# maxwellsh/DIGDriver

Hardware: NVIDIA B200
Metric: genome_bases_scanned_per_s (higher is better)
Workload: dtype u8 bases -> int32 counts; f64 p-values

## Files before the change

digdriver_b200/_lib.py:

```python
import ctypes
import os

_PKG_DIR = os.path.dirname(os.path.abspath(__file__))
LIB_PATH = os.environ.get("DIG_LIB_PATH") or os.path.join(_PKG_DIR, "libdigb200.so")

_c = ctypes
_P = _c.c_void_p
_I64 = _c.c_int64
_I = _c.c_int
_U64 = _c.c_uint64
_D = _c.c_double

SIGNATURES = {
    "dig_version": (_I, []),
    "dig_last_error": (_c.c_char_p, []),
    "dig_device_sm_count": (_I, []),
    "dig_packed_words": (_I64, [_I64]),
    "dig_nmask_words": (_I64, [_I64]),
    "dig_pack_genome": (_I, [_P, _I64, _P, _P, _P, _P]),
    "dig_scan_workspace_bytes": (_I64, [_I64]),
    "dig_count_contexts": (_I, [_P, _P, _I64, _P, _P, _P, _P, _P, _P, _I64, _I, _I, _P, _P, _P, _P]),
    "dig_count_contexts_fused53": (_I, [_P, _P, _I64, _P, _P, _P, _P, _P, _I64, _P, _P, _P, _P, _P, _P]),
    "dig_narrow_counts_u16": (_I, [_P, _I64, _P, _P, _P]),
    "dig_peer_broadcast": (_I, [_P, _I64, _P, _I, _P]),
    "dig_nmask_fill_runs": (_I, [_P, _I64, _P, _I64, _I64, _P]),
    "dig_nmask_summary": (_I, [_P, _I64, _I64, _P, _P]),
    "dig_tabulate_capacity": (_I64, [_I64]),
    "dig_tabulate_elements_workspace_bytes": (_I64, [_I64]),
    "dig_tabulate_genes_workspace_bytes": (_I64, [_I64]),
    "dig_synth_genome": (_I, [_P, _I64, _I64, _U64, _I, _P]),
    "dig_mutation_contexts": (_I, [_P, _P, _I64, _P, _P, _P, _P, _P, _I64, _I, _I, _P, _P]),
    "dig_substitution_counts": (_I, [_P, _P, _I64, _I, _I, _P, _P]),
    "dig_count_hits": (_I, [_P, _P, _P, _P, _I64, _P, _P, _I64, _P, _P]),
    "dig_tabulate_elements": (_I, [_P, _P, _P, _P, _I64, _P, _P, _P, _P, _I64, _P, _P, _P, _I64, _I64, _P,
                                   _I64, _I64, _I64, _P, _P, _I, _P]),
    "dig_site_counts": (_I, [_P, _P, _I64, _I64, _I, _P, _P]),
    "dig_tabulate_genes": (_I, [_P, _P, _P, _I64, _P, _P, _I64, _I64, _I64, _P, _P, _P, _P]),
    "dig_element_transfer": (_I, [_P, _P, _P, _P, _P, _I64, _I64, _I, _P, _P, _P, _P, _P, _P, _P, _I64, _I, _P,
                                  _P, _P, _I, _I, _P, _P, _P, _P, _P, _P, _P, _P, _P, _P]),
    "dig_nb_pvalue_greater_midp": (_I, [_P, _P, _P, _I64, _P, _P]),
    "dig_nb_burden_test": (_I, [_P, _P, _P, _P, _I64, _P, _P, _P]),
    "dig_fisher_combine2": (_I, [_P, _P, _I64, _P, _P]),
    "dig_sequence_freq": (_I, [_P, _P, _I, _P, _P]),
    "dig_size_ratio": (_I, [_P, _P, _I64, _P, _P]),
    "dig_gene_scale_sums": (_I, [_P, _P, _P, _P, _P, _P, _I64, _I64, _P, _P]),
    "dig_gene_burden_test": (_I, [_P, _P, _P, _P, _P, _P, _I64, _P, _D, _D, _P, _P]),
    "dig_gene_dnds_sel": (_I, [_P, _P, _P, _P, _I64, _P, _P]),
    "dig_selection_coefficient": (_I, [_P, _P, _P, _P, _P, _I64, _P, _P, _P]),
    "dig_window_denominators": (_I, [_P, _P, _I64, _P, _P, _P]),
    "dig_site_test": (_I, [_P, _P, _P, _P, _P, _I64, _I64, _I, _P, _P, _P, _P, _P, _P, _P, _D, _P, _P, _P, _P, _P]),
    "dig_region_prob_norm": (_I, [_P, _P, _I64, _I, _P, _P]),
    "dig_position_obs": (_I, [_P, _I64, _P, _P, _P, _P, _P, _I64, _I, _I, _I, _P, _I64, _P, _P]),
    "dig_position_test": (_I, [_P, _P, _I64, _P, _P, _P, _P, _P, _I64, _I, _I, _P, _P, _P, _P, _I, _P, _P, _P, _P,
                               _P, _P, _P]),
    "dig_nb_pvalue_exact": (_I, [_P, _P, _P, _I64, _P, _P]),
    "dig_nb_pvalue_variant": (_I, [_I, _P, _P, _P, _P, _I64, _P, _P]),
    "dig_loglik": (_I, [_I, _P, _P, _P, _I64, _P, _P]),
    "dig_gene_llr_test": (_I, [_I, _P, _P, _P, _P, _P, _P, _I64, _P, _P]),
    "dig_element_region_counts": (_I, [_P, _P, _P, _P, _P, _I64, _I64, _I, _P, _P, _P, _I64, _I, _P, _P, _P, _P]),
    "dig_element_psum": (_I, [_P, _P, _P, _I64, _P, _P, _P]),
    "dig_overlap_count": (_I, [_P, _P, _P, _I64, _P, _P, _I64, _P, _P]),
    "dig_overlap_fill": (_I, [_P, _P, _P, _I64, _P, _P, _I64, _P, _P, _P, _P]),
    "dig_cds_substitution_table": (_I, [_P, _P, _I64, _P, _P, _I, _P, _P, _P, _P, _P, _I64, _P, _I, _P, _I, _P, _P,
                                        _P, _P]),
    "dig_annotate_snvs": (_I, [_P, _P, _I64, _P, _P, _I, _P, _P, _P, _P, _P, _I64, _P, _I, _P, _I, _P, _P, _P, _P,
                               _I64, _P, _P, _P]),
}



class ScanOpts(ctypes.Structure):
    _fields_ = [("workspace_d", _c.c_void_p), ("workspace_bytes", _c.c_int64), ("variant", _c.c_int32),
                ("totals_limit_kb", _c.c_uint32), ("tile_window", _c.c_int64), ("n_peer_counts3", _c.c_int32),
                ("nsum_offset_words", _c.c_int32), ("peer_counts3_d", _c.c_void_p * 8), ("mc_counts3_d", _c.c_void_p)]


SCAN_AUTO, SCAN_PER_BASE, SCAN_HEX_PLAIN, SCAN_HEX = 0, 1, 2, 3

_lib = None

KERNELS_PER_CALL = {
    "dig_pack_genome": 1, "dig_count_contexts": 1, "dig_count_contexts_fused53": 1, "dig_synth_genome": 1, "dig_mutation_contexts": 1,
    "dig_substitution_counts": 1, "dig_count_hits": 1, "dig_tabulate_elements": 3, "dig_tabulate_genes": 2, "dig_site_counts": 1,
    "dig_element_transfer": 1, "dig_nb_pvalue_greater_midp": 1, "dig_nb_burden_test": 1, "dig_fisher_combine2": 1,
    "dig_sequence_freq": 1, "dig_size_ratio": 1, "dig_gene_scale_sums": 1, "dig_gene_burden_test": 2,
    "dig_window_denominators": 1, "dig_site_test": 1, "dig_gene_dnds_sel": 1, "dig_selection_coefficient": 1, "dig_region_prob_norm": 1, "dig_position_obs": 1, "dig_position_test": 1, "dig_nb_pvalue_exact": 1,
    "dig_nb_pvalue_variant": 1, "dig_loglik": 1, "dig_gene_llr_test": 1, "dig_overlap_count": 1, "dig_overlap_fill": 1,
    "dig_element_region_counts": 1, "dig_element_psum": 1, "dig_narrow_counts_u16": 1, "dig_peer_broadcast": 1, "dig_nmask_fill_runs": 1,
    "dig_nmask_summary": 1, "dig_cds_substitution_table": 1, "dig_annotate_snvs": 1,
}
launch_count = 0


class DigError(RuntimeError):
    pass


def load():
    global _lib
    if _lib is not None:
        return _lib
    if not os.path.exists(LIB_PATH):
        raise DigError(
            "libdigb200.so not found at %s: the CUDA extension is required (no CPU fallback). "
            "Build it with `python -m digdriver_b200.build`." % LIB_PATH)
    lib = ctypes.CDLL(LIB_PATH)
    for name, (res, args) in SIGNATURES.items():
        fn = getattr(lib, name)
        fn.restype = res
        fn.argtypes = args
    _lib = lib
    return lib


def check(rc, what=""):
    if rc != 0:
        msg = load().dig_last_error()
        raise DigError("%s failed with code %d: %s" % (what or "libdigb200 call", rc, (msg or b"").decode()))


def call(name, *args):
    global launch_count
    fn = getattr(load(), name)
    check(fn(*args), name)
    launch_count += KERNELS_PER_CALL.get(name, 0)
```

digdriver_b200/csrc/api.cu:

```cuda
#include <stdarg.h>
#include <string.h>

#include "dig_common.cuh"

namespace dig {

static thread_local char g_err[512] = "";

void set_error(const char *fmt, ...)
{
    va_list ap;
    va_start(ap, fmt);
    vsnprintf(g_err, sizeof(g_err), fmt, ap);
    va_end(ap);
}

int sm_count()
{
    static thread_local int cached_dev = -1;
    static thread_local int cached = 0;
    int dev = 0;
    if (cudaGetDevice(&dev) != cudaSuccess) return 148;
    if (dev != cached_dev) {
        int n = 0;
        if (cudaDeviceGetAttribute(&n, cudaDevAttrMultiProcessorCount, dev) != cudaSuccess || n <= 0) n = 148;
        cached = n;
        cached_dev = dev;
    }
    return cached;
}

}

extern "C" {

int dig_version(void) { return 100; }

const char *dig_last_error(void) { return dig::g_err; }

int dig_device_sm_count(void) { return dig::sm_count(); }

}
```

digdriver_b200/csrc/dig_common.cuh:

```cuda
#pragma once
#include <cuda_runtime.h>
#include <stdint.h>
#include <stdio.h>

#include "../../include/dig_b200.h"

namespace dig {

void set_error(const char *fmt, ...);
int sm_count();

#define DIG_CHECK_ARG(cond, msg)                           \
    do {                                                   \
        if (!(cond)) {                                     \
            dig::set_error("%s: %s", __func__, msg);       \
            return DIG_ERR_ARG;                            \
        }                                                  \
    } while (0)

#define DIG_CHECK_LAUNCH()                                                          \
    do {                                                                            \
        cudaError_t e__ = cudaGetLastError();                                       \
        if (e__ != cudaSuccess) {                                                   \
            dig::set_error("%s: CUDA error: %s", __func__, cudaGetErrorString(e__)); \
            return DIG_ERR_CUDA;                                                    \
        }                                                                           \
    } while (0)

#define DIG_CUDA(call)                                                              \
    do {                                                                            \
        cudaError_t e__ = (call);                                                   \
        if (e__ != cudaSuccess) {                                                   \
            dig::set_error("%s: %s failed: %s", __func__, #call, cudaGetErrorString(e__)); \
            return DIG_ERR_CUDA;                                                    \
        }                                                                           \
    } while (0)

__host__ __device__ __forceinline__ uint64_t mix64(uint64_t z)
{
    z += 0x9E3779B97F4A7C15ull;
    z = (z ^ (z >> 30)) * 0xBF58476D1CE4E5B9ull;
    z = (z ^ (z >> 27)) * 0x94D049BB133111EBull;
    return z ^ (z >> 31);
}

}
```

digdriver_b200/csrc/genetest.cu:

```cuda
#include <cooperative_groups.h>

#include "nb_math.cuh"

namespace {

using namespace dig_nb;

constexpr int SUMS_CLUSTER = 8;
__global__ void __cluster_dims__(SUMS_CLUSTER, 1, 1) __launch_bounds__(1024) gene_scale_sums_kernel(
    const double *__restrict__ mu, const double *__restrict__ sigma, const double *__restrict__ P,
    const double *__restrict__ pi_indel, const int64_t *__restrict__ obs, const uint8_t *__restrict__ cgc,
    int64_t tp53, int64_t n, double *__restrict__ sums)
{
    __shared__ double sh[3][1024];
    cooperative_groups::cluster_group cluster = cooperative_groups::this_cluster();
    const unsigned int rank = cluster.block_rank();
    double a0 = 0.0, a1 = 0.0, a2 = 0.0;
#pragma unroll 4
    for (int64_t g = (int64_t)rank * 1024 + threadIdx.x; g < n; g += (int64_t)SUMS_CLUSTER * 1024) {
        const double m = mu[g], s = sigma[g];
        const double t0 = m * P[g * 4 + 0];
        if (g != tp53 && !isnan(t0)) a0 += t0;
        if (cgc == nullptr || !cgc[g]) {
            const double alpha = (m * m) / (s * s);
            const double theta = (s * s) / m;
            const double t1 = pi_indel[g] * alpha * theta;
            if (!isnan(t1)) a1 += t1;
            a2 += (double)obs[g * 5 + 4];
        }
    }
    sh[0][threadIdx.x] = a0;
    sh[1][threadIdx.x] = a1;
    sh[2][threadIdx.x] = a2;
    __syncthreads();
    for (int o = 512; o > 0; o >>= 1) {
        if (threadIdx.x < o) {
            sh[0][threadIdx.x] += sh[0][threadIdx.x + o];
            sh[1][threadIdx.x] += sh[1][threadIdx.x + o];
            sh[2][threadIdx.x] += sh[2][threadIdx.x + o];
        }
        __syncthreads();
    }
    cluster.sync();
    if (rank == 0 && threadIdx.x < 3) {
        double acc = 0.0;
        for (unsigned int r = 0; r < (unsigned int)SUMS_CLUSTER; ++r) acc += *cluster.map_shared_rank(&sh[threadIdx.x][0], r);
        sums[threadIdx.x] = acc;
    }
    cluster.sync();
}

__global__ void __launch_bounds__(128) gene_test_kernel(
    const double *__restrict__ mu, const double *__restrict__ sigma, const double *__restrict__ P,
    const double *__restrict__ pi_indel, const int64_t *__restrict__ obs, const int64_t *__restrict__ nsamp,
    int64_t n, const double *__restrict__ sums, double n_syn,
    double scale_factor, double *__restrict__ out)
{
    const int64_t stride = (int64_t)gridDim.x * blockDim.x;
    const double cj = isnan(scale_factor) ? (isnan(n_syn) ? sums[3] : n_syn) / sums[0] : scale_factor;
    const double t_indel = sums[2] / sums[1];
    for (int64_t i = (int64_t)blockIdx.x * blockDim.x + threadIdx.x; i < n * 13; i += stride) {
        const int t = (int)(i / n);
        const int64_t g = i - (int64_t)t * n;
        const double m = mu[g], s = sigma[g];
        const double alpha = (m * m) / (s * s);
        const double theta0 = (s * s) / m;
        const double p_syn = P[g * 4 + 0], p_mis = P[g * 4 + 1], p_nons = P[g * 4 + 2], p_spl = P[g * 4 + 3];
        const double p_trunc = p_nons + p_spl;
        const double p_nonsyn = p_mis + p_trunc;
        double pi, k, theta;
        if (t == 12) {
            pi = pi_indel[g];
            k = (double)obs[g * 5 + 4];
            theta = theta0 * t_indel;
        } else {
            const int c = t % 6;
            pi = c == 0 ? p_syn : c == 1 ? p_mis : c == 2 ? p_nons : c == 3 ? p_spl : c == 4 ? p_trunc : p_nonsyn;
            theta = theta0 * cj;
            if (t < 6) {
                const double o0 = (double)obs[g * 5 + 0], o1 = (double)obs[g * 5 + 1], o2 = (double)obs[g * 5 + 2],
                             o3 = (double)obs[g * 5 + 3];
                k = c == 0 ? o0 : c == 1 ? o1 : c == 2 ? o2 : c == 3 ? o3 : c == 4 ? o2 + o3 : o1 + (o2 + o3);
            } else {
                k = (double)nsamp[g * 7 + (c < 4 ? c : c)];
            }
        }
        const double expv = __dmul_rn(__dmul_rn(alpha, theta), pi);
        const double p = __ddiv_rn(1.0, __dadd_rn(__dmul_rn(theta, pi), 1.0));
        const double pval = nb_midp(k, alpha, p);
        if (t < 6) {
            out[(int64_t)t * n + g] = expv;
            out[(int64_t)(6 + t) * n + g] = pval;
        } else if (t < 12) {
            out[(int64_t)(6 + t) * n + g] = pval;
        } else {
            out[18 * n + g] = expv;
            out[19 * n + g] = pval;
        }
        if (t == 0) {
            out[21 * n + g] = alpha;
            out[22 * n + g] = theta;
            out[23 * n + g] = theta0 * t_indel;
            out[24 * n + g] = pi_indel[g];
            out[25 * n + g] = p_trunc;
            out[26 * n + g] = p_nonsyn;
        }
    }
}

__global__ void __launch_bounds__(256) gene_fisher_kernel(int64_t n, double *__restrict__ out)
{
    const int64_t stride = (int64_t)gridDim.x * blockDim.x;
    for (int64_t g = (int64_t)blockIdx.x * blockDim.x + threadIdx.x; g < n; g += stride)
        out[20 * n + g] = fisher2(out[(6 + 4) * n + g], out[19 * n + g]);
}

__global__ void __launch_bounds__(256) seq_freq_kernel(const unsigned long long *__restrict__ counts,
                                                       const unsigned long long *__restrict__ totals, int n_sub,
                                                       double *__restrict__ freq)
{
    const int j = blockIdx.x * blockDim.x + threadIdx.x;
    if (j < n_sub) freq[j] = (double)counts[j] / (double)totals[j / 3];
}

__global__ void __launch_bounds__(256) size_ratio_kernel(const int64_t *__restrict__ num, const int64_t *__restrict__ den, int64_t n,
                                                         double *__restrict__ out)
{
    const int64_t i = (int64_t)blockIdx.x * blockDim.x + threadIdx.x;
    if (i < n) out[i] = __ddiv_rn((double)num[i], (double)den[i]);
}

}

extern "C" {

int dig_size_ratio(const int64_t *num_d, const int64_t *den_d, int64_t n, double *out_d, void *stream)
{
    DIG_CHECK_ARG(n >= 0, "negative size");
    if (n == 0) return DIG_OK;
    DIG_CHECK_ARG(num_d && den_d && out_d, "null pointer");
    size_ratio_kernel<<<(unsigned)((n + 255) / 256), 256, 0, (cudaStream_t)stream>>>(num_d, den_d, n, out_d);
    DIG_CHECK_LAUNCH();
    return DIG_OK;
}

int dig_sequence_freq(const unsigned long long *subst_counts_d, const unsigned long long *ctx_totals_d, int n_ctx,
                      double *freq_d, void *stream)
{
    DIG_CHECK_ARG(n_ctx > 0 && subst_counts_d && ctx_totals_d && freq_d, "bad arguments");
    const int n_sub = 3 * n_ctx;
    seq_freq_kernel<<<(n_sub + 255) / 256, 256, 0, (cudaStream_t)stream>>>(subst_counts_d, ctx_totals_d, n_sub, freq_d);
    DIG_CHECK_LAUNCH();
    return DIG_OK;
}

int dig_gene_scale_sums(const double *mu_d, const double *sigma_d, const double *p_d, const double *pi_indel_d,
                        const int64_t *obs_d, const uint8_t *cgc_mask_d, int64_t tp53, int64_t n_gene,
                        double *sums_d, void *stream)
{
    DIG_CHECK_ARG(n_gene >= 0 && sums_d, "bad arguments");
    DIG_CHECK_ARG(n_gene == 0 || (mu_d && sigma_d && p_d && pi_indel_d && obs_d), "null pointer");
    gene_scale_sums_kernel<<<SUMS_CLUSTER, 1024, 0, (cudaStream_t)stream>>>(mu_d, sigma_d, p_d, pi_indel_d, obs_d, cgc_mask_d,
                                                                 tp53, n_gene, sums_d);
    DIG_CHECK_LAUNCH();
    return DIG_OK;
}

int dig_gene_burden_test(const double *mu_d, const double *sigma_d, const double *p_d, const double *pi_indel_d,
                         const int64_t *obs_d, const int64_t *nsamp_d, int64_t n_gene, const double *sums_d,
                         double n_syn, double scale_factor, double *out_d, void *stream)
{
    DIG_CHECK_ARG(n_gene >= 0, "negative size");
    if (n_gene == 0) return DIG_OK;
    DIG_CHECK_ARG(mu_d && sigma_d && p_d && pi_indel_d && obs_d && nsamp_d && sums_d && out_d, "null pointer");
    cudaStream_t st = (cudaStream_t)stream;
    int64_t blocks = (n_gene * 13 + 127) / 128;
    const int64_t cap = (int64_t)dig::sm_count() * 32;
    if (blocks > cap) blocks = cap;
    gene_test_kernel<<<(unsigned)blocks, 128, 0, st>>>(mu_d, sigma_d, p_d, pi_indel_d, obs_d, nsamp_d, n_gene, sums_d,
                                                       n_syn, scale_factor, out_d);
    DIG_CHECK_LAUNCH();
    gene_fisher_kernel<<<(unsigned)((n_gene + 255) / 256), 256, 0, st>>>(n_gene, out_d);
    DIG_CHECK_LAUNCH();
    return DIG_OK;
}

}

namespace {

using namespace dig_nb;

__device__ inline double ll_nb(double k, double alpha, double theta)
{
    const double p = __ddiv_rn(1.0, __dadd_rn(1.0, theta));
    const double q = 1.0 - p;
    if (isnan(p) || isnan(k) || isnan(alpha)) return __longlong_as_double(0x7ff8000000000000LL);
    if (q <= 0.0) return k == 0.0 ? 0.0 : -INFINITY;
    if (p <= 0.0) return -INFINITY;
    return log_nb_density(k, alpha, p, q);
}

__global__ void __launch_bounds__(128) gene_dnds_sel_kernel(const double *__restrict__ alpha,
                                                            const double *__restrict__ theta,
                                                            const double *__restrict__ pi,
                                                            const double *__restrict__ obs,
                                                            int64_t n, double *__restrict__ out)
{
    const int64_t stride = (int64_t)gridDim.x * blockDim.x;
    for (int64_t g = (int64_t)blockIdx.x * blockDim.x + threadIdx.x; g < n; g += stride) {
        const double a = alpha[g], t = theta[g];
        double P[6], O[6], E[6];
#pragma unroll
        for (int j = 0; j < 6; ++j) {
            P[j] = pi[g * 6 + j];
            O[j] = obs[g * 6 + j];
            E[j] = __dmul_rn(__dmul_rn(a, t), P[j]);
            out[(int64_t)j * n + g] = E[j];
        }
        const double th_syn = __dmul_rn(t, P[0]);
        double tml = __ddiv_rn(__dadd_rn(__dadd_rn(O[0], a), -1.0), __dadd_rn(1.0, __ddiv_rn(1.0, th_syn)));
        if (a <= 1.0) {
            const double lo = __dmul_rn(a, th_syn);
            tml = tml > lo ? tml : lo;
        }
        const double ratio = __ddiv_rn(tml, E[0]);
        const double mrf = ratio > 1e-10 ? ratio : 1e-10;
        out[6 * n + g] = tml;
        out[7 * n + g] = mrf;
#pragma unroll
        for (int j = 0; j < 6; ++j) {
            const double eml = __dmul_rn(E[j], mrf);
            out[(int64_t)(8 + j) * n + g] = eml;
            const double p = __ddiv_rn(1.0, __dadd_rn(__ddiv_rn(eml, a), 1.0));
            out[(int64_t)(14 + j) * n + g] = nb_midp(O[j], a, p);
        }
        const int cls[3] = {0, 1, 4};
        double l0[3], l1[3];
#pragma unroll
        for (int c = 0; c < 3; ++c) {
            const int j = cls[c];
            l0[c] = ll_nb(O[j], a, __dmul_rn(__dmul_rn(t, P[j]), mrf));
            l1[c] = ll_nb(O[j], a, __ddiv_rn(O[j], a));
        }
        const double ll0 = __dadd_rn(__dadd_rn(l0[0], l0[1]), l0[2]);
        const double ll_syn = __dadd_rn(__dadd_rn(l1[0], l0[1]), l0[2]);
        const double ll_mis = __dadd_rn(__dadd_rn(l0[0], l1[1]), l0[2]);
        const double ll_tr = __dadd_rn(__dadd_rn(l0[0], l0[1]), l1[2]);
        const double ll_ns = __dadd_rn(__dadd_rn(l0[0], l1[1]), l1[2]);
        out[20 * n + g] = chi2_sf(-2.0 * (ll0 - ll_syn), 1);
        out[21 * n + g] = chi2_sf(-2.0 * (ll0 - ll_mis), 1);
        out[22 * n + g] = chi2_sf(-2.0 * (ll0 - ll_tr), 1);
        out[23 * n + g] = chi2_sf(-2.0 * (ll0 - ll_ns), 2);
    }
}

__global__ void __launch_bounds__(128) selection_coef_kernel(const double *__restrict__ obs, const double *__restrict__ ex,
                                                             const double *__restrict__ alpha,
                                                             const double *__restrict__ theta,
                                                             const double *__restrict__ pi, int64_t n,
                                                             double *__restrict__ sel, double *__restrict__ pval)
{
    const int64_t stride = (int64_t)gridDim.x * blockDim.x;
    for (int64_t g = (int64_t)blockIdx.x * blockDim.x + threadIdx.x; g < n; g += stride) {
        const double s = __ddiv_rn(__dadd_rn(obs[g], 1e-16), __dadd_rn(ex[g], 1e-16));
        sel[g] = s;
        if (pval) {
            const double tp = __dmul_rn(theta[g], pi[g]);
            const double ll0 = ll_nb(obs[g], alpha[g], tp);
            const double ll1 = ll_nb(obs[g], alpha[g], __dmul_rn(tp, s));
            pval[g] = chi2_sf(-2.0 * (ll0 - ll1), 1);
        }
    }
}

}

extern "C" int dig_gene_dnds_sel(const double *alpha_d, const double *theta_d, const double *pi6_d, const double *obs6_d,
                                 int64_t n_gene, double *out_d, void *stream)
{
    DIG_CHECK_ARG(n_gene >= 0, "negative size");
    if (n_gene == 0) return DIG_OK;
    DIG_CHECK_ARG(alpha_d && theta_d && pi6_d && obs6_d && out_d, "null pointer");
    int64_t blocks = (n_gene + 127) / 128;
    gene_dnds_sel_kernel<<<(unsigned)blocks, 128, 0, (cudaStream_t)stream>>>(alpha_d, theta_d, pi6_d, obs6_d, n_gene,
                                                                            out_d);
    DIG_CHECK_LAUNCH();
    return DIG_OK;
}

extern "C" int dig_selection_coefficient(const double *obs_d, const double *exp_d, const double *alpha_d,
                                         const double *theta_d, const double *pi_d, int64_t n, double *sel_d,
                                         double *pval_d, void *stream)
{
    DIG_CHECK_ARG(n >= 0, "negative size");
    if (n == 0) return DIG_OK;
    DIG_CHECK_ARG(obs_d && exp_d && sel_d, "null pointer");
    DIG_CHECK_ARG(pval_d == nullptr || (alpha_d && theta_d && pi_d), "p-values need alpha, theta and pi");
    int64_t blocks = (n + 127) / 128;
    selection_coef_kernel<<<(unsigned)blocks, 128, 0, (cudaStream_t)stream>>>(obs_d, exp_d, alpha_d, theta_d, pi_d, n,
                                                                             sel_d, pval_d);
    DIG_CHECK_LAUNCH();
    return DIG_OK;
}

namespace {

__global__ void __launch_bounds__(128) gene_llr_kernel(int model, const double *__restrict__ alpha,
                                                       const double *__restrict__ theta,
                                                       const double *__restrict__ pi,
                                                       const double *__restrict__ obs,
                                                       const double *__restrict__ mrfold, const double *__restrict__ t_syn,
                                                       int64_t n, double *__restrict__ out)
{
    const int64_t stride = (int64_t)gridDim.x * blockDim.x;
    for (int64_t g = (int64_t)blockIdx.x * blockDim.x + threadIdx.x; g < n; g += stride) {
        double r[4];
        llr_row(model, alpha[g], theta[g], pi + g * 3, obs + g * 3, mrfold[g], t_syn ? t_syn[g] : 0.0, r);
#pragma unroll
        for (int j = 0; j < 4; ++j) out[(int64_t)j * n + g] = r[j];
    }
}

}

extern "C" int dig_gene_llr_test(int model, const double *alpha_d, const double *theta_d, const double *pi3_d,
                                 const double *obs3_d, const double *mrfold_d, const double *t_syn_d, int64_t n,
                                 double *out_d, void *stream)
{
    DIG_CHECK_ARG(n >= 0, "negative size");
    DIG_CHECK_ARG(model == DIG_LLR_NB || model == DIG_LLR_GAMMA_POISSON, "unknown model");
    if (n == 0) return DIG_OK;
    DIG_CHECK_ARG(alpha_d && theta_d && pi3_d && obs3_d && mrfold_d && out_d, "null pointer");
    DIG_CHECK_ARG(model == DIG_LLR_NB || t_syn_d, "the gamma-Poisson model needs T_SYN");
    int64_t blocks = (n + 127) / 128;
    gene_llr_kernel<<<(unsigned)blocks, 128, 0, (cudaStream_t)stream>>>(model, alpha_d, theta_d, pi3_d, obs3_d, mrfold_d,
                                                                       t_syn_d, n, out_d);
    DIG_CHECK_LAUNCH();
    return DIG_OK;
}
```

digdriver_b200/csrc/mutctx.cu:

```cuda
#include "dig_common.cuh"

namespace {

__global__ void __launch_bounds__(256) mutctx_kernel(
    const uint32_t *__restrict__ p2, const uint32_t *__restrict__ nmask, int64_t last_p, int64_t last_m,
    const int64_t *__restrict__ chrom_off, const int64_t *__restrict__ chrom_len,
    const int32_t *__restrict__ mut_chrom, const int64_t *__restrict__ mut_start,
    const uint8_t *__restrict__ mut_ref, int64_t n_mut, int n_up, int n_down, int32_t *__restrict__ ctx_out)
{
    const int klen = n_up + n_down + 1;
    const int64_t stride = (int64_t)gridDim.x * blockDim.x;
    for (int64_t i = (int64_t)blockIdx.x * blockDim.x + threadIdx.x; i < n_mut; i += stride) {
        const int32_t c = mut_chrom[i];
        const int64_t p = mut_start[i];
        const int64_t L = __ldg(chrom_len + c);
        const int64_t off = __ldg(chrom_off + c);
        int32_t ctx = -1;
        if (p - n_up >= 0 && p + n_down < L) {
            const int64_t f = off + p - n_up;
            const int64_t w = f >> 4, m = f >> 5;
            const unsigned long long pk = ((unsigned long long)__ldg(p2 + w) << 32) | __ldg(p2 + (w < last_p ? w + 1 : last_p));
            const unsigned long long mk = ((unsigned long long)__ldg(nmask + m) << 32) | __ldg(nmask + (m < last_m ? m + 1 : last_m));
            const uint32_t key = (uint32_t)(pk >> (64 - 2 * ((int)(f & 15) + klen))) & ((1u << (2 * klen)) - 1u);
            const uint32_t bad = (uint32_t)(mk >> (64 - ((int)(f & 31) + klen))) & ((1u << klen) - 1u);
            const uint32_t base = (key >> (2 * n_down)) & 3u;
            const bool base_n = ((bad >> n_down) & 1u) != 0u;
            auto mismatch = [&](int64_t row) -> bool {
                const uint32_t ref = mut_ref[row];
                return ref > 3u || base_n || base != ref;
            };
            bool dropped = mismatch(i);
            for (int64_t j = i - 1; !dropped && j >= 0 && mut_chrom[j] == c && mut_start[j] == p; --j)
                dropped = mismatch(j);
            if (!dropped && bad == 0u) ctx = (int32_t)key;
        }
        ctx_out[i] = ctx;
    }
}

__global__ void __launch_bounds__(256) subst_hist_kernel(const int32_t *__restrict__ ctx,
                                                         const uint8_t *__restrict__ alt, int64_t n, int n_down,
                                                         int n_bins, unsigned long long *__restrict__ counts)
{
    extern __shared__ unsigned int sh[];
    for (int k = threadIdx.x; k < n_bins; k += blockDim.x) sh[k] = 0u;
    __syncthreads();
    const int64_t stride = (int64_t)gridDim.x * blockDim.x;
    for (int64_t i = (int64_t)blockIdx.x * blockDim.x + threadIdx.x; i < n; i += stride) {
        const int32_t c = ctx[i];
        const uint32_t a = alt[i];
        if (c < 0 || a > 3u) continue;
        const uint32_t ref = ((uint32_t)c >> (2 * n_down)) & 3u;
        if (a == ref) continue;
        atomicAdd(sh + 3 * c + (int)(a > ref ? a - 1u : a), 1u);
    }
    __syncthreads();
    for (int k = threadIdx.x; k < n_bins; k += blockDim.x)
        if (sh[k]) atomicAdd(counts + k, (unsigned long long)sh[k]);
}

}

extern "C" int dig_substitution_counts(const int32_t *ctx_d, const uint8_t *alt_d, int64_t n, int n_up, int n_down,
                                       unsigned long long *counts_d, void *stream)
{
    DIG_CHECK_ARG(n >= 0, "negative size");
    DIG_CHECK_ARG(n_up >= 0 && n_down >= 0 && n_up + n_down <= 5, "unsupported context size");
    DIG_CHECK_ARG(counts_d != nullptr, "null pointer");
    const int n_bins = 3 << (2 * (n_up + n_down + 1));
    cudaStream_t st = (cudaStream_t)stream;
    DIG_CUDA(cudaMemsetAsync(counts_d, 0, (size_t)n_bins * sizeof(unsigned long long), st));
    if (n == 0) return DIG_OK;
    DIG_CHECK_ARG(ctx_d && alt_d, "null pointer");
    int64_t blocks = (n + 255) / 256;
    const int64_t cap = (int64_t)dig::sm_count() * 4;
    if (blocks > cap) blocks = cap;
    subst_hist_kernel<<<(unsigned)blocks, 256, (size_t)n_bins * sizeof(unsigned int), st>>>(ctx_d, alt_d, n, n_down,
                                                                                          n_bins, counts_d);
    DIG_CHECK_LAUNCH();
    return DIG_OK;
}

extern "C" int dig_mutation_contexts(const uint32_t *packed2_d, const uint32_t *nmask_d, int64_t n_bases,
                                     const int64_t *chrom_off_d, const int64_t *chrom_len_d,
                                     const int32_t *mut_chrom_d, const int64_t *mut_start_d,
                                     const uint8_t *mut_ref_d, int64_t n_mut, int n_up, int n_down,
                                     int32_t *ctx_out_d, void *stream)
{
    DIG_CHECK_ARG(n_mut >= 0 && n_bases >= 0, "negative size");
    DIG_CHECK_ARG(n_up >= 0 && n_down >= 0 && n_up + n_down <= 14, "unsupported context size");
    if (n_mut == 0) return DIG_OK;
    DIG_CHECK_ARG(packed2_d && nmask_d && chrom_off_d && chrom_len_d && mut_chrom_d && mut_start_d && mut_ref_d &&
                      ctx_out_d,
                  "null pointer");
    int64_t blocks = (n_mut + 255) / 256;
    const int64_t cap = (int64_t)dig::sm_count() * 32;
    if (blocks > cap) blocks = cap;
    mutctx_kernel<<<(unsigned)blocks, 256, 0, (cudaStream_t)stream>>>(
        packed2_d, nmask_d, (((n_bases + 31) >> 5) << 1) - 1, ((n_bases + 31) >> 5) - 1, chrom_off_d, chrom_len_d,
        mut_chrom_d, mut_start_d, mut_ref_d, n_mut, n_up, n_down, ctx_out_d);
    DIG_CHECK_LAUNCH();
    return DIG_OK;
}
```

digdriver_b200/csrc/obs.cu:

```cuda
#include "dig_common.cuh"

namespace {

__device__ __forceinline__ int64_t upper_bound_ge(const int64_t *__restrict__ a, int64_t n, int64_t v)
{
    int64_t lo = 0, hi = n;
    while (lo < hi) {
        const int64_t mid = (lo + hi) >> 1;
        if (__ldg(a + mid) < v) lo = mid + 1;
        else hi = mid;
    }
    return lo;
}

template <typename F>
__device__ __forceinline__ void for_each_hit(const int64_t *__restrict__ bks, const int64_t *__restrict__ bke,
                                             const int64_t *__restrict__ pmax, const int32_t *__restrict__ belt,
                                             int64_t n_blk, int64_t ks, int64_t ke, F f)
{
    if (ke <= ks) return;
    const int64_t hi = upper_bound_ge(bks, n_blk, ke);
    for (int64_t idx = hi - 1; idx >= 0; --idx) {
        if (__ldg(pmax + idx) <= ks) break;
        if (__ldg(bke + idx) <= ks) continue;
        const int32_t e = __ldg(belt + idx);
        bool dup = false;
        for (int64_t j = hi - 1; j > idx && !dup; --j) dup = (__ldg(belt + j) == e) && (__ldg(bke + j) > ks);
        if (!dup) f(e);
    }
}

__global__ void __launch_bounds__(256) count_hits_kernel(
    const int64_t *__restrict__ bks, const int64_t *__restrict__ bke, const int64_t *__restrict__ pmax,
    const int32_t *__restrict__ belt, int64_t n_blk, const int64_t *__restrict__ mks,
    const int64_t *__restrict__ mke, int64_t n_mut, unsigned long long *n_hits)
{
    const int64_t stride = (int64_t)gridDim.x * blockDim.x;
    unsigned long long local = 0;
    for (int64_t i = (int64_t)blockIdx.x * blockDim.x + threadIdx.x; i < n_mut; i += stride)
        for_each_hit(bks, bke, pmax, belt, n_blk, mks[i], mke[i], [&](int32_t) { ++local; });
#pragma unroll
    for (int o = 16; o > 0; o >>= 1) local += __shfl_xor_sync(0xffffffffu, local, o);
    if ((threadIdx.x & 31) == 0 && local) atomicAdd(n_hits, local);
}

__device__ __forceinline__ int64_t table_slot(unsigned long long *keys, int64_t capacity, unsigned long long key)
{
    const int64_t mask = capacity - 1;
    int64_t slot = (int64_t)(dig::mix64(key) & (unsigned long long)mask);
    for (int64_t probes = 0; probes < capacity; ++probes) {
        const unsigned long long prev = atomicCAS(keys + slot, 0ull, key);
        if (prev == 0ull || prev == key) return slot;
        slot = (slot + 1) & mask;
    }
    return -1;
}

__global__ void __launch_bounds__(256) elt_insert_kernel(
    const int64_t *__restrict__ bks, const int64_t *__restrict__ bke, const int64_t *__restrict__ pmax,
    const int32_t *__restrict__ belt, int64_t n_blk, const int64_t *__restrict__ mks,
    const int64_t *__restrict__ mke, const int32_t *__restrict__ msample, const uint8_t *__restrict__ mindel,
    int64_t n_mut, unsigned long long *keys, uint32_t *snv, uint32_t *indel, int64_t capacity, int32_t *status)
{
    const int64_t stride = (int64_t)gridDim.x * blockDim.x;
    for (int64_t i = (int64_t)blockIdx.x * blockDim.x + threadIdx.x; i < n_mut; i += stride) {
        const unsigned long long sample = (unsigned long long)(uint32_t)msample[i];
        const bool is_indel = mindel[i] != 0;
        for_each_hit(bks, bke, pmax, belt, n_blk, mks[i], mke[i], [&](int32_t e) {
            const unsigned long long key = (((unsigned long long)(uint32_t)e << 32) | sample) + 1ull;
            const int64_t slot = table_slot(keys, capacity, key);
            if (slot < 0) {
                *status = 1;
                return;
            }
            atomicAdd((is_indel ? indel : snv) + slot, 1u);
        });
    }
}

__global__ void __launch_bounds__(256) elt_sample_totals_kernel(const unsigned long long *__restrict__ keys,
                                                                const uint32_t *__restrict__ snv,
                                                                const uint32_t *__restrict__ indel, int64_t capacity,
                                                                int rows_mode, unsigned long long *sample_tot)
{
    const int64_t stride = (int64_t)gridDim.x * blockDim.x;
    for (int64_t s = (int64_t)blockIdx.x * blockDim.x + threadIdx.x; s < capacity; s += stride) {
        const unsigned long long key = keys[s];
        if (key == 0ull) continue;
        const uint32_t sample = (uint32_t)((key - 1ull) & 0xFFFFFFFFull);
        atomicAdd(sample_tot + sample, rows_mode ? 1ull : (unsigned long long)snv[s] + (unsigned long long)indel[s]);
    }
}

__global__ void __launch_bounds__(256) elt_finalize_kernel(const unsigned long long *__restrict__ keys,
                                                           const uint32_t *__restrict__ snv,
                                                           const uint32_t *__restrict__ indel, int64_t capacity,
                                                           const unsigned long long *__restrict__ sample_tot,
                                                           int64_t max_per_sample, int64_t max_per_elt_sample,
                                                           int64_t n_elt, int64_t *obs)
{
    const int64_t stride = (int64_t)gridDim.x * blockDim.x;
    for (int64_t s = (int64_t)blockIdx.x * blockDim.x + threadIdx.x; s < capacity; s += stride) {
        const unsigned long long key = keys[s];
        if (key == 0ull) continue;
        const uint32_t sample = (uint32_t)((key - 1ull) & 0xFFFFFFFFull);
        const int64_t e = (int64_t)((key - 1ull) >> 32);
        if (e >= n_elt) continue;
        if ((int64_t)sample_tot[sample] > max_per_sample) continue;
        int64_t a = snv[s], b = indel[s];
        if (a > max_per_elt_sample) a = max_per_elt_sample;
        if (b > max_per_elt_sample) b = max_per_elt_sample;
        atomicAdd(reinterpret_cast<unsigned long long *>(obs + 3 * e + 0), 1ull);
        if (a) atomicAdd(reinterpret_cast<unsigned long long *>(obs + 3 * e + 1), (unsigned long long)a);
        if (b) atomicAdd(reinterpret_cast<unsigned long long *>(obs + 3 * e + 2), (unsigned long long)b);
    }
}

__global__ void __launch_bounds__(256) gene_insert_kernel(const int32_t *__restrict__ mgene,
                                                          const int32_t *__restrict__ msample,
                                                          const uint8_t *__restrict__ mclass, int64_t n_mut,
                                                          unsigned long long *keys, uint32_t *cnt, int64_t capacity,
                                                          int32_t *status)
{
    const int64_t stride = (int64_t)gridDim.x * blockDim.x;
    for (int64_t i = (int64_t)blockIdx.x * blockDim.x + threadIdx.x; i < n_mut; i += stride) {
        const uint32_t cls = mclass[i];
        const int32_t g = mgene[i];
        if (cls > 4u || g < 0) continue;
        const unsigned long long key =
            (((unsigned long long)(uint32_t)g << 32) | (unsigned long long)(uint32_t)msample[i]) + 1ull;
        const int64_t slot = table_slot(keys, capacity, key);
        if (slot < 0) {
            *status = 1;
            continue;
        }
        atomicAdd(cnt + slot * 5 + cls, 1u);
    }
}

__global__ void __launch_bounds__(256) gene_finalize_kernel(const unsigned long long *__restrict__ keys,
                                                            const uint32_t *__restrict__ cnt, int64_t capacity,
                                                            int64_t cap_per, int64_t n_gene, int64_t *obs,
                                                            int64_t *nsamp)
{
    const int64_t stride = (int64_t)gridDim.x * blockDim.x;
    for (int64_t s = (int64_t)blockIdx.x * blockDim.x + threadIdx.x; s < capacity; s += stride) {
        const unsigned long long key = keys[s];
        if (key == 0ull) continue;
        const int64_t g = (int64_t)((key - 1ull) >> 32);
        if (g >= n_gene) continue;
        int64_t c[5];
#pragma unroll
        for (int j = 0; j < 5; ++j) c[j] = cnt[s * 5 + j];
#pragma unroll
        for (int j = 0; j < 5; ++j) {
            const int64_t v = c[j] > cap_per ? cap_per : c[j];
            if (v) atomicAdd(reinterpret_cast<unsigned long long *>(obs + 5 * g + j), (unsigned long long)v);
        }
        const bool flags[7] = {c[0] > 0, c[1] > 0, c[2] > 0, c[3] > 0, (c[2] + c[3]) > 0, (c[1] + c[2] + c[3]) > 0,
                               c[4] > 0};
#pragma unroll
        for (int j = 0; j < 7; ++j)
            if (flags[j]) atomicAdd(reinterpret_cast<unsigned long long *>(nsamp + 7 * g + j), 1ull);
    }
}

__global__ void __launch_bounds__(256) site_counts_kernel(const int32_t *__restrict__ elt, const int32_t *__restrict__ sub,
                                                          int64_t n, int64_t n_elt, int n_sub,
                                                          unsigned long long *__restrict__ L)
{
    const int64_t stride = (int64_t)gridDim.x * blockDim.x;
    for (int64_t i = (int64_t)blockIdx.x * blockDim.x + threadIdx.x; i < n; i += stride) {
        const int32_t e = elt[i], j = sub[i];
        if (e >= 0 && e < n_elt && j >= 0 && j < n_sub) atomicAdd(L + (int64_t)e * n_sub + j, 1ull);
    }
}

inline unsigned grid_for(int64_t n)
{
    int64_t blocks = (n + 255) / 256;
    const int64_t cap = (int64_t)dig::sm_count() * 16;
    if (blocks > cap) blocks = cap;
    return (unsigned)(blocks < 1 ? 1 : blocks);
}

__global__ void __launch_bounds__(256) overlap_count_kernel(
    const int64_t *__restrict__ bks, const int64_t *__restrict__ bke, const int64_t *__restrict__ pmax, int64_t n_blk,
    const int64_t *__restrict__ mks, const int64_t *__restrict__ mke, int64_t n_mut, int64_t *__restrict__ n_pairs)
{
    const int64_t stride = (int64_t)gridDim.x * blockDim.x;
    for (int64_t i = (int64_t)blockIdx.x * blockDim.x + threadIdx.x; i < n_mut; i += stride) {
        const int64_t ks = mks[i], ke = mke[i];
        int64_t c = 0;
        if (ke > ks) {
            const int64_t hi = upper_bound_ge(bks, n_blk, ke);
            for (int64_t idx = hi - 1; idx >= 0; --idx) {
                if (__ldg(pmax + idx) <= ks) break;
                c += __ldg(bke + idx) > ks;
            }
        }
        n_pairs[i] = c;
    }
}

__global__ void __launch_bounds__(256) overlap_fill_kernel(
    const int64_t *__restrict__ bks, const int64_t *__restrict__ bke, const int64_t *__restrict__ pmax, int64_t n_blk,
    const int64_t *__restrict__ mks, const int64_t *__restrict__ mke, int64_t n_mut,
    const int64_t *__restrict__ pair_off, int64_t *__restrict__ pair_mut, int64_t *__restrict__ pair_blk)
{
    const int64_t stride = (int64_t)gridDim.x * blockDim.x;
    for (int64_t i = (int64_t)blockIdx.x * blockDim.x + threadIdx.x; i < n_mut; i += stride) {
        const int64_t ks = mks[i], ke = mke[i];
        if (ke <= ks) continue;
        int64_t w = pair_off[i + 1];
        const int64_t hi = upper_bound_ge(bks, n_blk, ke);
        for (int64_t idx = hi - 1; idx >= 0; --idx) {
            if (__ldg(pmax + idx) <= ks) break;
            if (__ldg(bke + idx) <= ks) continue;
            --w;
            pair_mut[w] = i;
            pair_blk[w] = idx;
        }
    }
}

inline bool is_pow2(int64_t v) { return v > 0 && (v & (v - 1)) == 0; }

}

extern "C" {

int64_t dig_tabulate_capacity(int64_t n_pairs)
{
    if (n_pairs < 0) n_pairs = 0;
    int64_t cap = 1024;
    while (cap < 2 * n_pairs + 16) cap <<= 1;
    return cap;
}
int64_t dig_tabulate_elements_workspace_bytes(int64_t n_pairs) { return dig_tabulate_capacity(n_pairs) * 16; }
int64_t dig_tabulate_genes_workspace_bytes(int64_t n_mut) { return dig_tabulate_capacity(n_mut) * 28; }

int dig_count_hits(const int64_t *blk_kstart_d, const int64_t *blk_kend_d, const int64_t *blk_pmax_d,
                   const int32_t *blk_elt_d, int64_t n_blk, const int64_t *mut_kstart_d,
                   const int64_t *mut_kend_d, int64_t n_mut, unsigned long long *n_hits_d, void *stream)
{
    DIG_CHECK_ARG(n_blk >= 0 && n_mut >= 0, "negative size");
    DIG_CHECK_ARG(n_hits_d != nullptr, "null pointer");
    if (n_blk == 0 || n_mut == 0) return DIG_OK;
    DIG_CHECK_ARG(blk_kstart_d && blk_kend_d && blk_pmax_d && blk_elt_d && mut_kstart_d && mut_kend_d, "null pointer");
    count_hits_kernel<<<grid_for(n_mut), 256, 0, (cudaStream_t)stream>>>(blk_kstart_d, blk_kend_d, blk_pmax_d,
                                                                         blk_elt_d, n_blk, mut_kstart_d, mut_kend_d,
                                                                         n_mut, n_hits_d);
    DIG_CHECK_LAUNCH();
    return DIG_OK;
}

int dig_tabulate_elements(const int64_t *blk_kstart_d, const int64_t *blk_kend_d, const int64_t *blk_pmax_d,
                          const int32_t *blk_elt_d, int64_t n_blk, const int64_t *mut_kstart_d,
                          const int64_t *mut_kend_d, const int32_t *mut_sample_d, const uint8_t *mut_isindel_d,
                          int64_t n_mut, unsigned long long *tab_key_d, uint32_t *tab_snv_d, uint32_t *tab_indel_d,
                          int64_t capacity, int64_t n_sample, unsigned long long *sample_tot_d,
                          int64_t max_muts_per_sample, int64_t max_per_elt_per_sample, int64_t n_elt,
                          int64_t *obs_d, int32_t *status_d, int sample_rows_mode, void *stream)
{
    DIG_CHECK_ARG(n_blk >= 0 && n_mut >= 0 && n_elt >= 0 && n_sample >= 0, "negative size");
    DIG_CHECK_ARG(is_pow2(capacity), "capacity must be a power of two");
    DIG_CHECK_ARG(tab_key_d && tab_snv_d && tab_indel_d && status_d, "null pointer");
    DIG_CHECK_ARG((n_elt == 0 || obs_d) && (n_sample == 0 || sample_tot_d), "null pointer");
    cudaStream_t st = (cudaStream_t)stream;
    DIG_CUDA(cudaMemsetAsync(tab_key_d, 0, (size_t)capacity * sizeof(unsigned long long), st));
    DIG_CUDA(cudaMemsetAsync(tab_snv_d, 0, (size_t)capacity * sizeof(uint32_t), st));
    DIG_CUDA(cudaMemsetAsync(tab_indel_d, 0, (size_t)capacity * sizeof(uint32_t), st));
    DIG_CUDA(cudaMemsetAsync(status_d, 0, sizeof(int32_t), st));
    if (n_sample) DIG_CUDA(cudaMemsetAsync(sample_tot_d, 0, (size_t)n_sample * sizeof(unsigned long long), st));
    if (n_elt) DIG_CUDA(cudaMemsetAsync(obs_d, 0, (size_t)n_elt * 3 * sizeof(int64_t), st));
    if (n_blk == 0 || n_mut == 0) return DIG_OK;
    DIG_CHECK_ARG(blk_kstart_d && blk_kend_d && blk_pmax_d && blk_elt_d && mut_kstart_d && mut_kend_d &&
                      mut_sample_d && mut_isindel_d,
                  "null pointer");
    elt_insert_kernel<<<grid_for(n_mut), 256, 0, st>>>(blk_kstart_d, blk_kend_d, blk_pmax_d, blk_elt_d, n_blk,
                                                       mut_kstart_d, mut_kend_d, mut_sample_d, mut_isindel_d, n_mut,
                                                       tab_key_d, tab_snv_d, tab_indel_d, capacity, status_d);
    DIG_CHECK_LAUNCH();
    elt_sample_totals_kernel<<<grid_for(capacity), 256, 0, st>>>(tab_key_d, tab_snv_d, tab_indel_d, capacity,
                                                                 sample_rows_mode, sample_tot_d);
    DIG_CHECK_LAUNCH();
    elt_finalize_kernel<<<grid_for(capacity), 256, 0, st>>>(tab_key_d, tab_snv_d, tab_indel_d, capacity, sample_tot_d,
                                                            max_muts_per_sample, max_per_elt_per_sample, n_elt, obs_d);
    DIG_CHECK_LAUNCH();
    return DIG_OK;
}

int dig_tabulate_genes(const int32_t *mut_gene_d, const int32_t *mut_sample_d, const uint8_t *mut_class_d,
                       int64_t n_mut, unsigned long long *tab_key_d, uint32_t *tab_cnt_d, int64_t capacity,
                       int64_t max_per_gene_per_sample, int64_t n_gene, int64_t *obs_d, int64_t *nsamp_d,
                       int32_t *status_d, void *stream)
{
    DIG_CHECK_ARG(n_mut >= 0 && n_gene >= 0, "negative size");
    DIG_CHECK_ARG(is_pow2(capacity), "capacity must be a power of two");
    DIG_CHECK_ARG(tab_key_d && tab_cnt_d && status_d && (n_gene == 0 || (obs_d && nsamp_d)), "null pointer");
    cudaStream_t st = (cudaStream_t)stream;
    DIG_CUDA(cudaMemsetAsync(tab_key_d, 0, (size_t)capacity * sizeof(unsigned long long), st));
    DIG_CUDA(cudaMemsetAsync(tab_cnt_d, 0, (size_t)capacity * 5 * sizeof(uint32_t), st));
    DIG_CUDA(cudaMemsetAsync(status_d, 0, sizeof(int32_t), st));
    if (n_gene) {
        DIG_CUDA(cudaMemsetAsync(obs_d, 0, (size_t)n_gene * 5 * sizeof(int64_t), st));
        DIG_CUDA(cudaMemsetAsync(nsamp_d, 0, (size_t)n_gene * 7 * sizeof(int64_t), st));
    }
    if (n_mut == 0) return DIG_OK;
    DIG_CHECK_ARG(mut_gene_d && mut_sample_d && mut_class_d, "null pointer");
    gene_insert_kernel<<<grid_for(n_mut), 256, 0, st>>>(mut_gene_d, mut_sample_d, mut_class_d, n_mut, tab_key_d,
                                                        tab_cnt_d, capacity, status_d);
    DIG_CHECK_LAUNCH();
    gene_finalize_kernel<<<grid_for(capacity), 256, 0, st>>>(tab_key_d, tab_cnt_d, capacity,
                                                             max_per_gene_per_sample, n_gene, obs_d, nsamp_d);
    DIG_CHECK_LAUNCH();
    return DIG_OK;
}

int dig_site_counts(const int32_t *site_elt_d, const int32_t *site_sub_d, int64_t n_site, int64_t n_elt, int n_sub,
                    unsigned long long *L_d, void *stream)
{
    DIG_CHECK_ARG(n_site >= 0 && n_elt >= 0 && n_sub > 0, "bad sizes");
    DIG_CHECK_ARG(n_elt == 0 || L_d, "null pointer");
    cudaStream_t st = (cudaStream_t)stream;
    if (n_elt) DIG_CUDA(cudaMemsetAsync(L_d, 0, (size_t)n_elt * n_sub * sizeof(unsigned long long), st));
    if (n_site == 0 || n_elt == 0) return DIG_OK;
    DIG_CHECK_ARG(site_elt_d && site_sub_d, "null pointer");
    site_counts_kernel<<<grid_for(n_site), 256, 0, st>>>(site_elt_d, site_sub_d, n_site, n_elt, n_sub, L_d);
    DIG_CHECK_LAUNCH();
    return DIG_OK;
}

int dig_overlap_count(const int64_t *blk_kstart_d, const int64_t *blk_kend_d, const int64_t *blk_pmax_d, int64_t n_blk,
                      const int64_t *mut_kstart_d, const int64_t *mut_kend_d, int64_t n_mut, int64_t *n_pairs_d,
                      void *stream)
{
    DIG_CHECK_ARG(n_blk >= 0 && n_mut >= 0, "negative size");
    if (n_mut == 0) return DIG_OK;
    DIG_CHECK_ARG(mut_kstart_d && mut_kend_d && n_pairs_d, "null pointer");
    DIG_CHECK_ARG(n_blk == 0 || (blk_kstart_d && blk_kend_d && blk_pmax_d), "null pointer");
    overlap_count_kernel<<<grid_for(n_mut), 256, 0, (cudaStream_t)stream>>>(blk_kstart_d, blk_kend_d, blk_pmax_d, n_blk,
                                                                            mut_kstart_d, mut_kend_d, n_mut, n_pairs_d);
    DIG_CHECK_LAUNCH();
    return DIG_OK;
}

int dig_overlap_fill(const int64_t *blk_kstart_d, const int64_t *blk_kend_d, const int64_t *blk_pmax_d, int64_t n_blk,
                     const int64_t *mut_kstart_d, const int64_t *mut_kend_d, int64_t n_mut, const int64_t *pair_off_d,
                     int64_t *pair_mut_d, int64_t *pair_blk_d, void *stream)
{
    DIG_CHECK_ARG(n_blk >= 0 && n_mut >= 0, "negative size");
    if (n_mut == 0 || n_blk == 0) return DIG_OK;
    DIG_CHECK_ARG(blk_kstart_d && blk_kend_d && blk_pmax_d && mut_kstart_d && mut_kend_d && pair_off_d, "null pointer");
    DIG_CHECK_ARG(pair_mut_d && pair_blk_d, "null pointer");
    overlap_fill_kernel<<<grid_for(n_mut), 256, 0, (cudaStream_t)stream>>>(blk_kstart_d, blk_kend_d, blk_pmax_d, n_blk,
                                                                           mut_kstart_d, mut_kend_d, n_mut, pair_off_d,
                                                                           pair_mut_d, pair_blk_d);
    DIG_CHECK_LAUNCH();
    return DIG_OK;
}

}
```

digdriver_b200/csrc/transfer.cu:

```cuda
#include "dig_common.cuh"

namespace {

constexpr int TW = 4;
constexpr int MAX_COHORT_PER_LANE = 2;

__device__ __forceinline__ double warp_sum(double v)
{
#pragma unroll
    for (int o = 16; o > 0; o >>= 1) v += __shfl_xor_sync(0xffffffffu, v, o);
    return v;
}

__device__ __forceinline__ int revcomp3(int c)
{
    const int b0 = (c >> 4) & 3, b1 = (c >> 2) & 3, b2 = c & 3;
    return ((3 - b2) << 4) | ((3 - b1) << 2) | (3 - b0);
}

__device__ __forceinline__ int64_t floor_div(int64_t a, int64_t b) { return a >= 0 ? a / b : -((-a + b - 1) / b); }
__device__ __forceinline__ int64_t ceil_div(int64_t a, int64_t b) { return a >= 0 ? (a + b - 1) / b : -((-a) / b); }

template <bool RC>
__global__ void __launch_bounds__(TW * 32, 8) transfer_kernel(
    const int32_t *__restrict__ elt_chrom, const int8_t *__restrict__ elt_strand,
    const int64_t *__restrict__ blk_ptr, const int64_t *__restrict__ blk_start,
    const int64_t *__restrict__ blk_end, int64_t n_elt, int64_t window, int n_chrom,
    const int64_t *__restrict__ win_map_off, const int32_t *__restrict__ win_map, const int32_t *__restrict__ win_counts,
    const double *__restrict__ y_pred, const double *__restrict__ stdv, const double *__restrict__ y_true,
    const uint8_t *__restrict__ flag, int64_t n_win, int n_cohort, const double *__restrict__ d_pr,
    const int32_t *__restrict__ blk_counts, const double *__restrict__ L_elt, int n_col, int span_words,
    double *__restrict__ mu_out, double *__restrict__ sigma_out, double *__restrict__ robs_out,
    uint8_t *__restrict__ flag_out, int64_t *__restrict__ r_size, int64_t *__restrict__ elt_size,
    double *__restrict__ p_out, int32_t *__restrict__ n_win_out, int32_t *__restrict__ status,
    int64_t *__restrict__ region_counts_out)
{
    extern __shared__ __align__(16) unsigned char smem_raw[];
    const int lane = threadIdx.x & 31;
    const int warp = threadIdx.x >> 5;
    const size_t per_warp = 128 * sizeof(double) + (size_t)span_words * sizeof(uint32_t);
    double *r64 = reinterpret_cast<double *>(smem_raw + warp * per_warp);
    double *l64 = r64 + 64;
    uint32_t *bitmap = reinterpret_cast<uint32_t *>(l64 + 64);

    const bool l4_aligned = (reinterpret_cast<uintptr_t>(L_elt) & 15u) == 0;
    const int64_t gwarp = (int64_t)blockIdx.x * TW + warp;
    const int64_t nwarps = (int64_t)gridDim.x * TW;

    for (int64_t e = gwarp; e < n_elt; e += nwarps) {
        const int64_t b0 = blk_ptr[e], b1 = blk_ptr[e + 1];
        const int32_t c = elt_chrom[e];
        const bool minus = elt_strand[e] < 0;
        int64_t wmin = INT64_MAX, wmax = INT64_MIN;
        for (int64_t b = b0 + lane; b < b1; b += 32) {
            const int64_t lo = floor_div(blk_start[b], window);
            const int64_t hi = ceil_div(blk_end[b], window);
            if (hi > lo) {
                wmin = lo < wmin ? lo : wmin;
                wmax = hi > wmax ? hi : wmax;
            }
        }
#pragma unroll
        for (int o = 16; o > 0; o >>= 1) {
            const int64_t a = __shfl_xor_sync(0xffffffffu, wmin, o);
            const int64_t b = __shfl_xor_sync(0xffffffffu, wmax, o);
            wmin = a < wmin ? a : wmin;
            wmax = b > wmax ? b : wmax;
        }
        const int64_t span = wmax > wmin ? wmax - wmin : 0;
        const int words = (int)((span + 31) >> 5);
        bool ok = true;
        if (words > span_words) {
            if (lane == 0) atomicMax(status, 3);
            ok = false;
        }
        if (ok) {
            for (int w = lane; w < words; w += 32) bitmap[w] = 0u;
            __syncwarp();
            for (int64_t b = b0 + lane; b < b1; b += 32) {
                const int64_t lo = floor_div(blk_start[b], window) - wmin;
                const int64_t hi = ceil_div(blk_end[b], window) - wmin;
                for (int64_t w = lo; w < hi;) {
                    const int word = (int)(w >> 5);
                    const int bit = (int)(w & 31);
                    const int64_t upto = ((int64_t)(word + 1) << 5) < hi ? ((int64_t)(word + 1) << 5) : hi;
                    const int nbits = (int)(upto - w);
                    const uint32_t m = (nbits >= 32 ? 0xFFFFFFFFu : ((1u << nbits) - 1u)) << bit;
                    atomicOr(bitmap + word, m);
                    w = upto;
                }
            }
            __syncwarp();
        }
        double r_lo = 0.0, r_hi = 0.0;
        double mu[MAX_COHORT_PER_LANE], var[MAX_COHORT_PER_LANE], ro[MAX_COHORT_PER_LANE];
        int fl[MAX_COHORT_PER_LANE];
#pragma unroll
        for (int q = 0; q < MAX_COHORT_PER_LANE; ++q) mu[q] = var[q] = ro[q] = 0.0, fl[q] = 0;
        int nw = 0;
        const bool chrom_ok = c >= 0 && c < n_chrom;
        const int64_t map0 = chrom_ok ? win_map_off[c] : 0;
        const int64_t map_n = chrom_ok ? win_map_off[c + 1] - map0 : 0;
        for (int w = 0; ok && w < words; ++w) {
            const uint32_t bits = bitmap[w];
            const int cnt = __popc(bits);
            if (cnt == 0) continue;
            int32_t my_row = -1;
            if (lane < cnt) {
                const int64_t wi = wmin + ((int64_t)w << 5) + (int64_t)__fns(bits, 0, lane + 1);
                my_row = (wi >= 0 && wi < map_n) ? __ldg(win_map + map0 + wi) : -1;
            }
            if (__any_sync(0xffffffffu, lane < cnt && my_row < 0) && lane == 0) atomicMax(status, 2);
            for (int k0 = 0; k0 < cnt; k0 += 4) {
                int32_t row[4], clo[4], chi[4];
#pragma unroll
                for (int u = 0; u < 4; ++u) {
                    row[u] = k0 + u < cnt ? __shfl_sync(0xffffffffu, my_row, (k0 + u) & 31) : -1;
                    clo[u] = chi[u] = 0;
                    if (row[u] >= 0) {
                        const int32_t *wc = win_counts + (int64_t)row[u] * 64;
                        clo[u] = __ldg(wc + lane);
                        chi[u] = __ldg(wc + lane + 32);
                    }
                }
#pragma unroll
                for (int u = 0; u < 4; ++u) {
                    if (row[u] < 0) continue;
                    ++nw;
                    r_lo += (double)clo[u];
                    r_hi += (double)chi[u];
                }
            }
            if (n_cohort == 1) {
                double yp = 0.0, sd = 0.0, yt = 0.0;
                int fg = 0;
                if (lane < cnt && my_row >= 0) {
                    yp = __ldg(y_pred + my_row);
                    sd = __ldg(stdv + my_row);
                    yt = __ldg(y_true + my_row);
                    fg = __ldg(flag + my_row) != 0;
                }
                for (int k = 0; k < cnt; ++k) {
                    const double a = __shfl_sync(0xffffffffu, yp, k), b = __shfl_sync(0xffffffffu, sd, k);
                    const double t = __shfl_sync(0xffffffffu, yt, k);
                    const int f = __shfl_sync(0xffffffffu, fg, k);
                    if (__shfl_sync(0xffffffffu, my_row, k) < 0) continue;
                    mu[0] += a;
                    var[0] = __dadd_rn(var[0], __dmul_rn(b, b));
                    ro[0] += t;
                    fl[0] |= f;
                }
            } else {
                for (int k = 0; k < cnt; ++k) {
                    const int32_t row = __shfl_sync(0xffffffffu, my_row, k);
                    if (row < 0) continue;
#pragma unroll
                    for (int q = 0; q < MAX_COHORT_PER_LANE; ++q) {
                        const int ci = lane + 32 * q;
                        if (ci < n_cohort) {
                            const int64_t o = (int64_t)ci * n_win + row;
                            const double s = __ldg(stdv + o);
                            mu[q] += __ldg(y_pred + o);
                            var[q] = __dadd_rn(var[q], __dmul_rn(s, s));
                            ro[q] += __ldg(y_true + o);
                            fl[q] |= __ldg(flag + o) != 0;
                        }
                    }
                }
            }
        }
        __syncwarp();
        if (!minus) {
            r64[lane] = r_lo;
            r64[lane + 32] = r_hi;
        } else {
            r64[revcomp3(lane)] = r_lo;
            r64[revcomp3(lane + 32)] = r_hi;
        }
        double l_lo = 0.0, l_hi = 0.0;
        int64_t gene_len = 0;
        if (blk_counts != nullptr) {
            for (int64_t b = b0; b < b1; ++b) {
                l_lo += (double)__ldg(blk_counts + b * 64 + lane);
                l_hi += (double)__ldg(blk_counts + b * 64 + lane + 32);
            }
            l64[lane] = l_lo;
            l64[lane + 32] = l_hi;
        } else {
            for (int64_t b = b0 + lane; b < b1; b += 32) gene_len += blk_end[b] - blk_start[b] + 1;
#pragma unroll
            for (int o = 16; o > 0; o >>= 1) gene_len += __shfl_xor_sync(0xffffffffu, gene_len, o);
        }
        __syncwarp();
        if (RC) {
            region_counts_out[e * 64 + lane] = (int64_t)r64[lane];
            region_counts_out[e * 64 + lane + 32] = (int64_t)r64[lane + 32];
        }
        const double rsum = warp_sum(r_lo + r_hi);
        const double lsum = warp_sum(l_lo + l_hi);

        for (int ci = 0; ci < n_cohort; ++ci) {
            const double *dp = d_pr + (int64_t)ci * 192;
            double part = 0.0;
#pragma unroll
            for (int t = 0; t < 6; ++t) {
                const int j = lane + 32 * t;
                part += __ldg(dp + j) * r64[j / 3];
            }
            const double denom = warp_sum(part);
            double wgt[6];
#pragma unroll
            for (int t = 0; t < 6; ++t) wgt[t] = __ldg(dp + lane + 32 * t) / denom;
            if (blk_counts == nullptr && n_col == 4 && l4_aligned) {
                const double2 *L2 = reinterpret_cast<const double2 *>(L_elt + (int64_t)e * 192 * 4);
                double2 la[6], lb[6];
#pragma unroll
                for (int t = 0; t < 6; ++t) {
                    la[t] = __ldg(L2 + 2 * (lane + 32 * t));
                    lb[t] = __ldg(L2 + 2 * (lane + 32 * t) + 1);
                }
                double a0 = 0.0, a1 = 0.0, a2 = 0.0, a3 = 0.0;
#pragma unroll
                for (int t = 0; t < 6; ++t) {
                    a0 += wgt[t] * la[t].x;
                    a1 += wgt[t] * la[t].y;
                    a2 += wgt[t] * lb[t].x;
                    a3 += wgt[t] * lb[t].y;
                }
                a0 = warp_sum(a0);
                a1 = warp_sum(a1);
                a2 = warp_sum(a2);
                a3 = warp_sum(a3);
                if (lane == 0) {
                    double *po = p_out + ((int64_t)ci * n_elt + e) * 4;
                    po[0] = a0;
                    po[1] = a1;
                    po[2] = a2;
                    po[3] = a3;
                }
            } else {
                for (int col = 0; col < n_col; ++col) {
                    double acc = 0.0;
#pragma unroll
                    for (int t = 0; t < 6; ++t) {
                        const int j = lane + 32 * t;
                        const double Lj = blk_counts != nullptr ? l64[j / 3]
                                                                : __ldg(L_elt + ((int64_t)e * 192 + j) * n_col + col);
                        acc += wgt[t] * Lj;
                    }
                    acc = warp_sum(acc);
                    if (lane == 0) p_out[((int64_t)ci * n_elt + e) * n_col + col] = acc;
                }
            }
        }
#pragma unroll
        for (int q = 0; q < MAX_COHORT_PER_LANE; ++q) {
            const int ci = lane + 32 * q;
            if (ci < n_cohort) {
                const int64_t o = (int64_t)ci * n_elt + e;
                mu_out[o] = mu[q];
                sigma_out[o] = sqrt(var[q]);
                robs_out[o] = ro[q];
                flag_out[o] = (uint8_t)fl[q];
            }
        }
        if (lane == 0) {
            if (!RC || r_size) r_size[e] = (int64_t)rsum;
            if (!RC || elt_size) elt_size[e] = blk_counts != nullptr ? (int64_t)lsum : gene_len;
            n_win_out[e] = nw;
        }
        __syncwarp();
    }
}

}

extern "C" int dig_element_transfer(const int32_t *elt_chrom_d, const int8_t *elt_strand_d, const int64_t *blk_ptr_d,
                                    const int64_t *blk_start_d, const int64_t *blk_end_d, int64_t n_elt,
                                    int64_t window, int n_chrom, const int64_t *win_map_off_d, const int32_t *win_map_d,
                                    const int32_t *win_counts_d, const double *y_pred_d, const double *std_d,
                                    const double *y_true_d, const uint8_t *flag_d, int64_t n_win, int n_cohort,
                                    const double *d_pr_d, const int32_t *blk_counts_d, const double *L_elt_d,
                                    int n_col, int max_span_windows, double *mu_d, double *sigma_d, double *r_obs_d,
                                    uint8_t *flag_out_d, int64_t *r_size_d, int64_t *elt_size_d, double *p_out_d,
                                    int32_t *n_win_out_d, int32_t *status_d, void *stream)
{
    DIG_CHECK_ARG(n_elt >= 0 && n_win >= 0 && window > 0 && n_chrom >= 0, "bad sizes");
    DIG_CHECK_ARG(n_cohort >= 1 && n_cohort <= 32 * MAX_COHORT_PER_LANE, "n_cohort must be in [1, 64] per call");
    DIG_CHECK_ARG((blk_counts_d != nullptr) != (L_elt_d != nullptr), "pass exactly one of blk_counts_d / L_elt_d");
    DIG_CHECK_ARG(blk_counts_d == nullptr || n_col == 1, "n_col must be 1 with blk_counts_d");
    DIG_CHECK_ARG(n_col >= 1 && max_span_windows >= 1, "bad n_col / max_span_windows");
    DIG_CHECK_ARG(status_d != nullptr, "null pointer");
    cudaStream_t st = (cudaStream_t)stream;
    DIG_CUDA(cudaMemsetAsync(status_d, 0, sizeof(int32_t), st));
    if (n_elt == 0) return DIG_OK;
    DIG_CHECK_ARG(elt_chrom_d && elt_strand_d && blk_ptr_d && blk_start_d && blk_end_d && win_map_off_d &&
                      win_map_d && win_counts_d && y_pred_d && std_d && y_true_d && flag_d && d_pr_d && mu_d &&
                      sigma_d && r_obs_d && flag_out_d && r_size_d && elt_size_d && p_out_d && n_win_out_d,
                  "null pointer");
    const int span_words = ((max_span_windows + 31) / 32 + 3) & ~3;
    const size_t smem = (size_t)TW * (128 * sizeof(double) + (size_t)span_words * sizeof(uint32_t));
    if (smem > 200 * 1024) {
        dig::set_error("dig_element_transfer: window span of %d windows needs %zu B of shared memory",
                       max_span_windows, smem);
        return DIG_ERR_UNSUPPORTED;
    }
    DIG_CUDA(cudaFuncSetAttribute(transfer_kernel<false>, cudaFuncAttributeMaxDynamicSharedMemorySize, (int)smem));
    int64_t blocks = (n_elt + TW - 1) / TW;
    const int64_t cap = (int64_t)dig::sm_count() * 64;
    if (blocks > cap) blocks = cap;
    transfer_kernel<false><<<(unsigned)blocks, TW * 32, smem, st>>>(
        elt_chrom_d, elt_strand_d, blk_ptr_d, blk_start_d, blk_end_d, n_elt, window, n_chrom, win_map_off_d, win_map_d,
        win_counts_d, y_pred_d, std_d, y_true_d, flag_d, n_win, n_cohort, d_pr_d, blk_counts_d, L_elt_d, n_col,
        span_words, mu_d, sigma_d, r_obs_d, flag_out_d, r_size_d, elt_size_d, p_out_d, n_win_out_d, status_d, nullptr);
    DIG_CHECK_LAUNCH();
    return DIG_OK;
}

extern "C" int dig_element_region_counts(const int32_t *elt_chrom_d, const int8_t *elt_strand_d, const int64_t *blk_ptr_d,
                                         const int64_t *blk_start_d, const int64_t *blk_end_d, int64_t n_elt,
                                         int64_t window, int n_chrom, const int64_t *win_map_off_d, const int32_t *win_map_d,
                                         const int32_t *win_counts_d, int64_t n_win, int max_span_windows,
                                         int64_t *region_counts_d, int32_t *n_win_out_d, int32_t *status_d, void *stream)
{
    DIG_CHECK_ARG(n_elt >= 0 && n_win >= 0 && window > 0 && max_span_windows >= 1 && n_chrom >= 0, "bad sizes");
    DIG_CHECK_ARG(status_d != nullptr, "null pointer");
    cudaStream_t st = (cudaStream_t)stream;
    DIG_CUDA(cudaMemsetAsync(status_d, 0, sizeof(int32_t), st));
    if (n_elt == 0) return DIG_OK;
    DIG_CHECK_ARG(elt_chrom_d && elt_strand_d && blk_ptr_d && blk_start_d && blk_end_d && win_map_off_d && win_map_d &&
                      win_counts_d && region_counts_d && n_win_out_d,
                  "null pointer");
    const int span_words = ((max_span_windows + 31) / 32 + 3) & ~3;
    const size_t smem = (size_t)TW * (128 * sizeof(double) + (size_t)span_words * sizeof(uint32_t));
    if (smem > 200 * 1024) {
        dig::set_error("dig_element_region_counts: window span of %d windows needs %zu B of shared memory",
                       max_span_windows, smem);
        return DIG_ERR_UNSUPPORTED;
    }
    DIG_CUDA(cudaFuncSetAttribute(transfer_kernel<true>, cudaFuncAttributeMaxDynamicSharedMemorySize, (int)smem));
    int64_t blocks = (n_elt + TW - 1) / TW;
    const int64_t cap = (int64_t)dig::sm_count() * 64;
    if (blocks > cap) blocks = cap;
    transfer_kernel<true><<<(unsigned)blocks, TW * 32, smem, st>>>(
        elt_chrom_d, elt_strand_d, blk_ptr_d, blk_start_d, blk_end_d, n_elt, window, n_chrom, win_map_off_d, win_map_d,
        win_counts_d, nullptr, nullptr, nullptr, nullptr, n_win, 0, nullptr, nullptr, nullptr, 0, span_words, nullptr,
        nullptr, nullptr, nullptr, nullptr, nullptr, nullptr, n_win_out_d, status_d, region_counts_d);
    DIG_CHECK_LAUNCH();
    return DIG_OK;
}

namespace {

__global__ void __launch_bounds__(128) element_psum_kernel(const double *__restrict__ L, const int64_t *__restrict__ R,
                                                           const double *__restrict__ d_pr, int64_t n_elt,
                                                           double *__restrict__ p_out, double *__restrict__ denom_out)
{
    const int lane = threadIdx.x & 31;
    const int64_t gwarp = ((int64_t)blockIdx.x * blockDim.x + threadIdx.x) >> 5;
    const int64_t nwarps = ((int64_t)gridDim.x * blockDim.x) >> 5;
    for (int64_t e = gwarp; e < n_elt; e += nwarps) {
        double part = 0.0;
#pragma unroll
        for (int t = 0; t < 6; ++t) {
            const int j = lane + 32 * t;
            part += __ldg(d_pr + j) * (double)__ldg(R + e * 192 + j);
        }
        const double denom = warp_sum(part);
        double acc = 0.0;
#pragma unroll
        for (int t = 0; t < 6; ++t) {
            const int j = lane + 32 * t;
            acc += (__ldg(d_pr + j) / denom) * __ldg(L + e * 192 + j);
        }
        acc = warp_sum(acc);
        if (lane == 0) {
            p_out[e] = acc;
            if (denom_out) denom_out[e] = denom;
        }
    }
}

}

extern "C" int dig_element_psum(const double *L_d, const int64_t *region_counts_d, const double *d_pr_d, int64_t n_elt,
                                double *p_out_d, double *denom_out_d, void *stream)
{
    DIG_CHECK_ARG(n_elt >= 0, "negative size");
    if (n_elt == 0) return DIG_OK;
    DIG_CHECK_ARG(L_d && region_counts_d && d_pr_d && p_out_d, "null pointer");
    int64_t blocks = (n_elt + 3) / 4;
    const int64_t cap = (int64_t)dig::sm_count() * 32;
    if (blocks > cap) blocks = cap;
    element_psum_kernel<<<(unsigned)blocks, 128, 0, (cudaStream_t)stream>>>(L_d, region_counts_d, d_pr_d, n_elt, p_out_d,
                                                                           denom_out_d);
    DIG_CHECK_LAUNCH();
    return DIG_OK;
}
```

digdriver_b200/kernels.py:

```python
import numpy as np
import torch

from . import _lib


def _stream(device, stream=None):
    st = stream if stream is not None else torch.cuda.current_stream(device)
    return st.cuda_stream


def _dev(x, dtype, device):
    if isinstance(x, torch.Tensor):
        return x.to(device=device, dtype=dtype).contiguous()
    return torch.from_numpy(np.ascontiguousarray(x)).to(device=device, dtype=dtype)


def _ptr(t):
    return t.data_ptr() if t is not None else None


def _tile_hint(reg_start, reg_end, tile_window):
    if tile_window is not None:
        return int(tile_window)
    if isinstance(reg_start, torch.Tensor) or isinstance(reg_end, torch.Tensor):
        return 0
    s, e = np.asarray(reg_start), np.asarray(reg_end)
    if s.size == 0:
        return 0
    w = int(e.flat[0]) - int(s.flat[0])
    return w if w > 0 and bool(np.all(e - s == w)) else 0


def _scan_opts(dev, n_reg, variant, totals_limit_kb, workspace, tile_window=0, peer_rows=None, mc_rows=None, genome=None):
    import ctypes
    if workspace is None and n_reg > 0:
        nbytes = int(_lib.load().dig_scan_workspace_bytes(int(n_reg)))
        workspace = torch.empty(nbytes, dtype=torch.uint8, device=dev)
    opts = _lib.ScanOpts(workspace.data_ptr() if workspace is not None else None,
                         workspace.numel() if workspace is not None else 0, int(variant), int(totals_limit_kb),
                         int(tile_window))
    if peer_rows:
        assert len(peer_rows) <= 8, "at most 8 peers"
        opts.n_peer_counts3 = len(peer_rows)
        for i, a in enumerate(peer_rows):
            opts.peer_counts3_d[i] = int(a)
        opts.mc_counts3_d = int(mc_rows) if mc_rows else None
    if genome is not None and getattr(genome, "nsum", None) is not None:
        assert genome.nsum.data_ptr() == genome.nmask.data_ptr() + 4 * genome.nsum_offset
        opts.nsum_offset_words = genome.nsum_offset
    return opts, ctypes.byref(opts), workspace


def peer_broadcast(src, dst_addrs, stream=None):
    import ctypes
    dev = src.device
    arr = (ctypes.c_void_p * len(dst_addrs))(*[int(a) for a in dst_addrs])
    with torch.cuda.device(dev):
        _lib.call("dig_peer_broadcast", src.data_ptr(), src.numel() * src.element_size(), arr, len(dst_addrs), _stream(dev, stream))


def scan_workspace(genome_or_device, n_reg):
    dev = getattr(genome_or_device, "device", genome_or_device)
    return torch.empty(int(_lib.load().dig_scan_workspace_bytes(int(n_reg))), dtype=torch.uint8, device=dev)


def count_contexts(genome, reg_chrom, reg_start, reg_end, n_up=1, n_down=1, strand=None,
                   want_totals=False, out=None, totals=None, stream=None, variant=_lib.SCAN_AUTO,
                   totals_limit_kb=0, workspace=None, tile_window=None, peer_rows=None, mc_rows=None):
    dev = genome.device
    rc = _dev(reg_chrom, torch.int32, dev)
    rs = _dev(reg_start, torch.int64, dev)
    re = _dev(reg_end, torch.int64, dev)
    st = _dev(strand, torch.int8, dev) if strand is not None else None
    n = rc.numel()
    K = 4 ** (n_up + n_down + 1)
    if out is None:
        out = torch.empty((n, K), dtype=torch.int32, device=dev)
    if want_totals and totals is None:
        totals = torch.zeros(K, dtype=torch.int64, device=dev)
    lane_bank = (n_up, n_down) in ((2, 2), (1, 1)) and st is None and variant == _lib.SCAN_AUTO
    opts, opts_ref, workspace = _scan_opts(dev, n if lane_bank else 0, variant, totals_limit_kb,
                                           workspace if lane_bank else None,
                                           _tile_hint(reg_start, reg_end, tile_window) if lane_bank else 0,
                                           peer_rows, mc_rows, genome)
    with torch.cuda.device(dev):
        _lib.call("dig_count_contexts", genome.packed2.data_ptr(), genome.nmask.data_ptr(), genome.n_bases,
                  genome.chrom_off_d.data_ptr(), genome.chrom_len_d.data_ptr(), rc.data_ptr(), rs.data_ptr(),
                  re.data_ptr(), _ptr(st), n, int(n_up), int(n_down), out.data_ptr(), _ptr(totals), opts_ref,
                  _stream(dev, stream))
    if lane_bank and n > 0:
        _lib.launch_count += 1
    return out, totals


def count_contexts_fused53(genome, reg_chrom, reg_start, reg_end, want_totals=False, out5=None, out3=None,
                           totals5=None, totals3=None, stream=None, variant=_lib.SCAN_AUTO, totals_limit_kb=0,
                           workspace=None, tile_window=None, peer_rows=None, mc_rows=None):
    dev = genome.device
    rc = _dev(reg_chrom, torch.int32, dev)
    rs = _dev(reg_start, torch.int64, dev)
    re = _dev(reg_end, torch.int64, dev)
    n = rc.numel()
    if out5 is None:
        out5 = torch.empty((n, 1024), dtype=torch.int32, device=dev)
    if out3 is None:
        out3 = torch.empty((n, 64), dtype=torch.int32, device=dev)
    if want_totals and totals5 is None:
        totals5 = torch.zeros(1024, dtype=torch.int64, device=dev)
        totals3 = torch.zeros(64, dtype=torch.int64, device=dev)
    lane_bank = variant == _lib.SCAN_AUTO
    opts, opts_ref, workspace = _scan_opts(dev, n if lane_bank else 0, variant, totals_limit_kb,
                                           workspace if lane_bank else None,
                                           _tile_hint(reg_start, reg_end, tile_window) if lane_bank else 0,
                                           peer_rows, mc_rows, genome)
    with torch.cuda.device(dev):
        _lib.call("dig_count_contexts_fused53", genome.packed2.data_ptr(), genome.nmask.data_ptr(), genome.n_bases,
                  genome.chrom_off_d.data_ptr(), genome.chrom_len_d.data_ptr(), rc.data_ptr(), rs.data_ptr(),
                  re.data_ptr(), n, out5.data_ptr(), out3.data_ptr(), _ptr(totals5), _ptr(totals3), opts_ref,
                  _stream(dev, stream))
    if lane_bank and n > 0:
        _lib.launch_count += 1
    return out5, out3, totals5, totals3


def mutation_contexts(genome, mut_chrom, mut_start, mut_ref, n_up=1, n_down=1, stream=None):
    dev = genome.device
    mc = _dev(mut_chrom, torch.int32, dev)
    ms = _dev(mut_start, torch.int64, dev)
    mr = _dev(mut_ref, torch.uint8, dev)
    out = torch.empty(mc.numel(), dtype=torch.int32, device=dev)
    with torch.cuda.device(dev):
        _lib.call("dig_mutation_contexts", genome.packed2.data_ptr(), genome.nmask.data_ptr(), genome.n_bases,
                  genome.chrom_off_d.data_ptr(), genome.chrom_len_d.data_ptr(), mc.data_ptr(), ms.data_ptr(),
                  mr.data_ptr(), mc.numel(), int(n_up), int(n_down), out.data_ptr(), _stream(dev, stream))
    return out


def nb_pvalue_greater_midp(k, alpha, p, device="cuda:0", stream=None):
    dev = torch.device(device)
    kd, ad, pd_ = (_dev(x, torch.float64, dev) for x in (k, alpha, p))
    out = torch.empty_like(kd)
    with torch.cuda.device(dev):
        _lib.call("dig_nb_pvalue_greater_midp", kd.data_ptr(), ad.data_ptr(), pd_.data_ptr(), kd.numel(),
                  out.data_ptr(), _stream(dev, stream))
    return out


def nb_burden_test(k, alpha, theta, pi, device="cuda:0", want_exp=True, stream=None):
    dev = torch.device(device)
    kd, ad, td, fd = (_dev(x, torch.float64, dev) for x in (k, alpha, theta, pi))
    pval = torch.empty_like(kd)
    exp = torch.empty_like(kd) if want_exp else None
    with torch.cuda.device(dev):
        _lib.call("dig_nb_burden_test", kd.data_ptr(), ad.data_ptr(), td.data_ptr(), fd.data_ptr(), kd.numel(),
                  _ptr(exp), pval.data_ptr(), _stream(dev, stream))
    return exp, pval


def fisher_combine2(p1, p2, device="cuda:0", stream=None):
    dev = torch.device(device)
    a, b = _dev(p1, torch.float64, dev), _dev(p2, torch.float64, dev)
    out = torch.empty_like(a)
    with torch.cuda.device(dev):
        _lib.call("dig_fisher_combine2", a.data_ptr(), b.data_ptr(), a.numel(), out.data_ptr(), _stream(dev, stream))
    return out


def _table_capacity(n_pairs):
    return int(_lib.load().dig_tabulate_capacity(int(n_pairs)))


def _check_status(status, what, sink=None):
    if sink is not None:
        sink.append((status, what))
        return
    code = int(status.item())
    if code == 1:
        raise _lib.DigError("%s: hash table overflow" % what)
    if code == 2:
        raise KeyError("%s: an element overlaps a window that is not in region_params "
                       "(the reference raises KeyError on the same input)" % what)
    if code == 3:
        raise _lib.DigError("%s: element window span exceeds the shared-memory bitmap" % what)
    if code != 0:
        raise _lib.DigError("%s: status %d" % (what, code))


def check_deferred(sink):
    pending, sink[:] = list(sink), []
    for status, what in pending:
        _check_status(status, what)


def tabulate_elements(blk_kstart, blk_kend, blk_elt, mut_kstart, mut_kend, mut_sample, mut_isindel,
                      n_elt, n_sample, max_muts_per_sample=10 ** 9, max_per_elt_per_sample=3 * 10 ** 9,
                      device="cuda:0", stream=None, sample_rows_mode=False, return_table=False, max_hits=None,
                      status_sink=None):
    dev = torch.device(device)
    bks = np.asarray(blk_kstart, dtype=np.int64)
    order = np.argsort(bks, kind="stable")
    bks = bks[order]
    bke = np.asarray(blk_kend, dtype=np.int64)[order]
    belt = np.asarray(blk_elt, dtype=np.int32)[order]
    pmax = np.maximum.accumulate(bke) if len(bke) else bke
    t = {k: _dev(v, dt, dev) for k, v, dt in (
        ("bks", bks, torch.int64), ("bke", bke, torch.int64), ("pmax", pmax, torch.int64), ("belt", belt, torch.int32),
        ("mks", mut_kstart, torch.int64), ("mke", mut_kend, torch.int64), ("ms", mut_sample, torch.int32),
        ("mi", mut_isindel, torch.uint8))}
    n_blk, n_mut = len(bks), t["mks"].numel()
    sptr = _stream(dev, stream)
    with torch.cuda.device(dev):
        if max_hits is None:
            n_hits = torch.zeros(1, dtype=torch.int64, device=dev)
            _lib.call("dig_count_hits", t["bks"].data_ptr(), t["bke"].data_ptr(), t["pmax"].data_ptr(),
                      t["belt"].data_ptr(), n_blk, t["mks"].data_ptr(), t["mke"].data_ptr(), n_mut, n_hits.data_ptr(), sptr)
            max_hits = int(n_hits.item())
        cap = _table_capacity(max_hits)
        keys = torch.empty(cap, dtype=torch.int64, device=dev)
        snv = torch.empty(cap, dtype=torch.int32, device=dev)
        ind = torch.empty(cap, dtype=torch.int32, device=dev)
        sample_tot = torch.empty(max(n_sample, 1), dtype=torch.int64, device=dev)
        obs = torch.empty((max(n_elt, 1), 3), dtype=torch.int64, device=dev)
        status = torch.zeros(1, dtype=torch.int32, device=dev)
        _lib.call("dig_tabulate_elements", t["bks"].data_ptr(), t["bke"].data_ptr(), t["pmax"].data_ptr(),
                  t["belt"].data_ptr(), n_blk, t["mks"].data_ptr(), t["mke"].data_ptr(), t["ms"].data_ptr(),
                  t["mi"].data_ptr(), n_mut, keys.data_ptr(), snv.data_ptr(), ind.data_ptr(), cap, n_sample,
                  sample_tot.data_ptr(), int(min(max_muts_per_sample, 2 ** 62)),
                  int(min(max_per_elt_per_sample, 2 ** 62)), n_elt, obs.data_ptr(), status.data_ptr(),
                  int(bool(sample_rows_mode)), sptr)
        _check_status(status, "dig_tabulate_elements", status_sink)
    if return_table:
        return obs[:n_elt], sample_tot[:n_sample], (keys, snv, ind)
    return obs[:n_elt], sample_tot[:n_sample]


def tabulate_genes(mut_gene, mut_sample, mut_class, n_gene, max_per_gene_per_sample=3 * 10 ** 9,
                   device="cuda:0", stream=None, status_sink=None):
    dev = torch.device(device)
    mg, ms, mc = _dev(mut_gene, torch.int32, dev), _dev(mut_sample, torch.int32, dev), _dev(mut_class, torch.uint8, dev)
    n_mut = mg.numel()
    cap = _table_capacity(n_mut)
    with torch.cuda.device(dev):
        keys = torch.empty(cap, dtype=torch.int64, device=dev)
        cnt = torch.empty((cap, 5), dtype=torch.int32, device=dev)
        obs = torch.empty((max(n_gene, 1), 5), dtype=torch.int64, device=dev)
        nsamp = torch.empty((max(n_gene, 1), 7), dtype=torch.int64, device=dev)
        status = torch.zeros(1, dtype=torch.int32, device=dev)
        _lib.call("dig_tabulate_genes", mg.data_ptr(), ms.data_ptr(), mc.data_ptr(), n_mut, keys.data_ptr(),
                  cnt.data_ptr(), cap, int(min(max_per_gene_per_sample, 2 ** 62)), n_gene, obs.data_ptr(),
                  nsamp.data_ptr(), status.data_ptr(), _stream(dev, stream))
        _check_status(status, "dig_tabulate_genes", status_sink)
    return obs[:n_gene], nsamp[:n_gene]


def element_transfer(elt_chrom, elt_strand, blk_ptr, blk_start, blk_end, window, win_map_off, win_map,
                     win_counts, y_pred, std, y_true, flag, d_pr, blk_counts=None, L_elt=None,
                     device="cuda:0", stream=None, max_span=None, status_sink=None):
    dev = torch.device(device)
    ec, es = _dev(elt_chrom, torch.int32, dev), _dev(elt_strand, torch.int8, dev)
    bp, bs, be = (_dev(x, torch.int64, dev) for x in (blk_ptr, blk_start, blk_end))
    wmo, wm = _dev(win_map_off, torch.int64, dev), _dev(win_map, torch.int32, dev)
    wc = _dev(win_counts, torch.int32, dev)
    yp, sd, yt = (_dev(x, torch.float64, dev).reshape(-1, wc.shape[0]) for x in (y_pred, std, y_true))
    fl = _dev(np.asarray(flag).astype(np.uint8) if not isinstance(flag, torch.Tensor) else flag.to(torch.uint8),
              torch.uint8, dev).reshape(-1, wc.shape[0])
    dp = _dev(d_pr, torch.float64, dev).reshape(-1, 192)
    n_cohort = dp.shape[0]
    assert yp.shape[0] == n_cohort and sd.shape[0] == n_cohort and yt.shape[0] == n_cohort and fl.shape[0] == n_cohort
    n_elt = ec.numel()
    n_win = wc.shape[0]
    if blk_counts is not None:
        bc, Le, n_col = _dev(blk_counts, torch.int32, dev), None, 1
    else:
        Le = _dev(L_elt, torch.float64, dev)
        Le = Le.reshape(n_elt, 192, -1)
        bc, n_col = None, Le.shape[2]
    if max_span is None:
        max_span = element_max_span(bp, bs, be, window)
    out = {
        "MU": torch.empty((n_cohort, n_elt), dtype=torch.float64, device=dev),
        "SIGMA": torch.empty((n_cohort, n_elt), dtype=torch.float64, device=dev),
        "R_OBS": torch.empty((n_cohort, n_elt), dtype=torch.float64, device=dev),
        "FLAG": torch.empty((n_cohort, n_elt), dtype=torch.uint8, device=dev),
        "R_SIZE": torch.empty(n_elt, dtype=torch.int64, device=dev),
        "ELT_SIZE": torch.empty(n_elt, dtype=torch.int64, device=dev),
        "P": torch.empty((n_cohort, n_elt, n_col), dtype=torch.float64, device=dev),
        "N_WIN": torch.empty(n_elt, dtype=torch.int32, device=dev),
    }
    status = torch.zeros(1, dtype=torch.int32, device=dev)
    with torch.cuda.device(dev):
        _lib.call("dig_element_transfer", ec.data_ptr(), es.data_ptr(), bp.data_ptr(), bs.data_ptr(), be.data_ptr(),
                  n_elt, int(window), int(wmo.numel()) - 1, wmo.data_ptr(), wm.data_ptr(), wc.data_ptr(), yp.data_ptr(),
                  sd.data_ptr(), yt.data_ptr(), fl.data_ptr(), n_win, n_cohort, dp.data_ptr(), _ptr(bc), _ptr(Le), n_col, max_span,
                  out["MU"].data_ptr(), out["SIGMA"].data_ptr(), out["R_OBS"].data_ptr(), out["FLAG"].data_ptr(),
                  out["R_SIZE"].data_ptr(), out["ELT_SIZE"].data_ptr(), out["P"].data_ptr(),
                  out["N_WIN"].data_ptr(), status.data_ptr(), _stream(dev, stream))
        _check_status(status, "dig_element_transfer", status_sink)
    return out


def element_max_span(blk_ptr, blk_start, blk_end, window):
    def host(x):
        return x.cpu().numpy() if isinstance(x, torch.Tensor) else np.asarray(x)
    bp_h, bs_h, be_h = host(blk_ptr).astype(np.int64), host(blk_start).astype(np.int64), host(blk_end).astype(np.int64)
    n_elt = len(bp_h) - 1
    max_span = 1
    if n_elt > 0 and len(bs_h):
        lo = np.floor_divide(bs_h, window)
        hi = -np.floor_divide(-be_h, window)
        owner = np.repeat(np.arange(n_elt), np.diff(bp_h))
        wmin = np.full(n_elt, np.iinfo(np.int64).max)
        wmax = np.full(n_elt, np.iinfo(np.int64).min)
        np.minimum.at(wmin, owner, lo)
        np.maximum.at(wmax, owner, hi)
        has = wmax > wmin
        if has.any():
            max_span = int((wmax[has] - wmin[has]).max())
    return max_span


def build_window_map(win_chrom_idx, win_start, window, n_chrom):
    wc = np.asarray(win_chrom_idx, dtype=np.int64)
    wn = np.asarray(win_start, dtype=np.int64) // int(window)
    per = np.zeros(n_chrom, dtype=np.int64)
    if len(wc):
        np.maximum.at(per, wc, wn + 1)
    off = np.zeros(n_chrom + 1, dtype=np.int64)
    off[1:] = np.cumsum(per)
    wmap = np.full(int(off[-1]), -1, dtype=np.int32)
    wmap[off[wc] + wn] = np.arange(len(wc), dtype=np.int32)
    return off, wmap


def substitution_counts(ctx, alt, n_up=1, n_down=1, stream=None, out=None):
    dev = ctx.device
    al = _dev(alt, torch.uint8, dev)
    if out is None:
        out = torch.empty(3 * 4 ** (n_up + n_down + 1), dtype=torch.int64, device=dev)
    assert out.dtype == torch.int64 and out.is_contiguous() and out.numel() == 3 * 4 ** (n_up + n_down + 1)
    with torch.cuda.device(dev):
        _lib.call("dig_substitution_counts", ctx.data_ptr(), al.data_ptr(), ctx.numel(), int(n_up), int(n_down),
                  out.data_ptr(), _stream(dev, stream))
    return out


def sequence_freq(subst_counts, ctx_totals, stream=None):
    dev = subst_counts.device
    n_ctx = ctx_totals.numel()
    out = torch.empty(3 * n_ctx, dtype=torch.float64, device=dev)
    with torch.cuda.device(dev):
        _lib.call("dig_sequence_freq", subst_counts.data_ptr(), ctx_totals.data_ptr(), n_ctx, out.data_ptr(),
                  _stream(dev, stream))
    return out


GENE_OUT_ROWS = (["EXP_" + c for c in ("SYN", "MIS", "NONS", "SPL", "TRUNC", "NONSYN")] +
                 ["PVAL_%s_BURDEN" % c for c in ("SYN", "MIS", "NONS", "SPL", "TRUNC", "NONSYN")] +
                 ["PVAL_%s_BURDEN_SAMPLE" % c for c in ("SYN", "MIS", "NONS", "SPL", "TRUNC", "NONSYN")] +
                 ["EXP_INDEL", "PVAL_INDEL_BURDEN", "PVAL_MUT_BURDEN", "ALPHA", "THETA", "THETA_INDEL", "Pi_INDEL",
                  "Pi_TRUNC", "Pi_NONSYN"])


def size_ratio(num, den, stream=None):
    dev = num.device
    assert num.dtype == torch.int64 and den.dtype == torch.int64 and num.is_contiguous() and den.is_contiguous()
    assert num.numel() == den.numel()
    out = torch.empty(num.shape, dtype=torch.float64, device=dev)
    with torch.cuda.device(dev):
        _lib.call("dig_size_ratio", num.data_ptr(), den.data_ptr(), num.numel(), out.data_ptr(), _stream(dev, stream))
    return out


def gene_scale_sums(mu, sigma, P, pi_indel, obs, cgc_mask=None, tp53=-1, stream=None):
    dev = mu.device
    sums = torch.empty(3, dtype=torch.float64, device=dev)
    cg = _dev(cgc_mask, torch.uint8, dev) if cgc_mask is not None else None
    with torch.cuda.device(dev):
        _lib.call("dig_gene_scale_sums", mu.data_ptr(), sigma.data_ptr(), P.data_ptr(), pi_indel.data_ptr(),
                  obs.data_ptr(), _ptr(cg), int(tp53), mu.numel(), sums.data_ptr(), _stream(dev, stream))
    return sums


def gene_burden_test(mu, sigma, P, pi_indel, obs, nsamp, sums, n_syn, scale_factor=None, stream=None):
    dev = mu.device
    E = mu.numel()
    out = torch.empty((len(GENE_OUT_ROWS), E), dtype=torch.float64, device=dev)
    with torch.cuda.device(dev):
        _lib.call("dig_gene_burden_test", mu.data_ptr(), sigma.data_ptr(), P.data_ptr(), pi_indel.data_ptr(),
                  obs.data_ptr(), nsamp.data_ptr(), E, sums.data_ptr(), float("nan") if n_syn is None else float(n_syn),
                  float("nan") if scale_factor is None else float(scale_factor), out.data_ptr(), _stream(dev, stream))
    return out


def site_counts(site_elt, site_sub, n_elt, n_sub=192, device="cuda:0", stream=None):
    dev = torch.device(device)
    se, ss = _dev(site_elt, torch.int32, dev), _dev(site_sub, torch.int32, dev)
    out = torch.empty((max(n_elt, 1), n_sub), dtype=torch.int64, device=dev)
    with torch.cuda.device(dev):
        _lib.call("dig_site_counts", se.data_ptr(), ss.data_ptr(), se.numel(), n_elt, n_sub, out.data_ptr(),
                  _stream(dev, stream))
    return out[:n_elt]


def nb_pvalue_exact(k, alpha, p, device="cuda:0", stream=None):
    dev = torch.device(device)
    kk, aa, pp = (_dev(x, torch.float64, dev).contiguous() for x in (k, alpha, p))
    out = torch.empty_like(kk)
    with torch.cuda.device(dev):
        _lib.call("dig_nb_pvalue_exact", kk.data_ptr(), aa.data_ptr(), pp.data_ptr(), kk.numel(), out.data_ptr(),
                  _stream(dev, stream))
    return out


def position_bins(genome, reg_chrom, reg_start, reg_end, n_up, n_down, binsize):
    rc = np.asarray(reg_chrom, dtype=np.int64)
    rs = np.asarray(reg_start, dtype=np.int64).copy()
    re = np.asarray(reg_end, dtype=np.int64)
    L = np.asarray(genome.chrom_len, dtype=np.int64)[rc]
    rs[rs < n_up] = n_up
    first = np.minimum(rs, L)
    last = np.minimum(re + n_down, L) - n_down
    n_pos = np.maximum(last - first, 0)
    n_bin = -(-n_pos // binsize)
    ptr = np.zeros(len(rc) + 1, dtype=np.int64)
    ptr[1:] = np.cumsum(n_bin)
    return first, n_pos, ptr


def position_test(genome, reg_chrom, reg_start, reg_end, mu, sigma, s_prob, mut_chrom, mut_start, n_up=2, n_down=2,
                  binsize=1, normed=True, want=("pt", "exp", "pos"), stream=None):
    dev = genome.device
    rc = _dev(reg_chrom, torch.int32, dev)
    rs = _dev(reg_start, torch.int64, dev)
    re = _dev(reg_end, torch.int64, dev)
    n_reg = rc.numel()
    K = 4 ** (n_up + n_down + 1)
    sp = _dev(s_prob, torch.float64, dev).contiguous()
    assert sp.numel() == K, "s_prob must have 4^(n_up+n_down+1) entries"
    mu_d, sg_d = _dev(mu, torch.float64, dev).contiguous(), _dev(sigma, torch.float64, dev).contiguous()
    assert mu_d.numel() == n_reg and sg_d.numel() == n_reg
    host = lambda x: x.cpu().numpy() if isinstance(x, torch.Tensor) else np.asarray(x)
    first, n_pos, ptr = position_bins(genome, host(reg_chrom), host(reg_start), host(reg_end), n_up, n_down, binsize)
    n_bin = int(ptr[-1])
    ptr_d = torch.from_numpy(ptr).to(dev)
    mk = (host(mut_chrom).astype(np.int64) << 32) | host(mut_start).astype(np.int64)
    mk_d = torch.from_numpy(np.sort(mk)).to(dev)
    sptr = _stream(dev, stream)
    out = {"bin_ptr": ptr, "n_pos": n_pos, "first": first}
    with torch.cuda.device(dev):
        norm = None
        if normed:
            counts, _ = count_contexts(genome, rc, rs, re, n_up, n_down, stream=stream)
            norm = torch.empty(n_reg, dtype=torch.float64, device=dev)
            _lib.call("dig_region_prob_norm", counts.data_ptr(), sp.data_ptr(), n_reg, K, norm.data_ptr(), sptr)
            out["norm"] = norm
        obs = torch.empty(max(n_bin, 1), dtype=torch.int32, device=dev)
        _lib.call("dig_position_obs", mk_d.data_ptr(), mk_d.numel(), genome.chrom_off_d.data_ptr(),
                  genome.chrom_len_d.data_ptr(), rc.data_ptr(), rs.data_ptr(), re.data_ptr(), n_reg, int(n_up),
                  int(n_down), int(binsize), ptr_d.data_ptr(), n_bin, obs.data_ptr(), sptr)
        pval = torch.empty(max(n_bin, 1), dtype=torch.float64, device=dev)
        extra = {k: (torch.empty(max(n_bin, 1), dtype=torch.float64, device=dev) if k in want else None)
                 for k in ("pt", "exp", "pos")}
        _lib.call("dig_position_test", genome.packed2.data_ptr(), genome.nmask.data_ptr(), genome.n_bases,
                  genome.chrom_off_d.data_ptr(), genome.chrom_len_d.data_ptr(), rc.data_ptr(), rs.data_ptr(),
                  re.data_ptr(), n_reg, int(n_up), int(n_down), sp.data_ptr(), _ptr(norm), mu_d.data_ptr(),
                  sg_d.data_ptr(), int(binsize), ptr_d.data_ptr(), obs.data_ptr(), pval.data_ptr(),
                  _ptr(extra["pt"]), _ptr(extra["exp"]), _ptr(extra["pos"]), sptr)
    out["pval"], out["obs"] = pval[:n_bin], obs[:n_bin]
    for k, v in extra.items():
        if v is not None:
            out[k] = v[:n_bin]
    return out


DNDS_CLASSES = ("SYN", "MIS", "NONS", "SPL", "TRUNC", "NONSYN")
DNDS_OUT_ROWS = (["EXP_%s" % c for c in DNDS_CLASSES] + ["T_SYN", "MRFOLD"] + ["EXP_%s_ML" % c for c in DNDS_CLASSES] +
                 ["PVAL_%s_BURDEN_DNDS" % c for c in DNDS_CLASSES] +
                 ["PVAL_SYN_SEL_NB", "PVAL_MIS_SEL_NB", "PVAL_TRUNC_SEL_NB", "PVAL_NONSYN_SEL_NB"])


def gene_dnds_sel(alpha, theta, pi6, obs6, device="cuda:0", stream=None):
    dev = torch.device(device)
    a, t = _dev(alpha, torch.float64, dev).contiguous(), _dev(theta, torch.float64, dev).contiguous()
    p6, o6 = _dev(pi6, torch.float64, dev).contiguous(), _dev(obs6, torch.float64, dev).contiguous()
    E = a.numel()
    assert p6.shape == (E, 6) and o6.shape == (E, 6)
    out = torch.empty((len(DNDS_OUT_ROWS), E), dtype=torch.float64, device=dev)
    with torch.cuda.device(dev):
        _lib.call("dig_gene_dnds_sel", a.data_ptr(), t.data_ptr(), p6.data_ptr(), o6.data_ptr(), E, out.data_ptr(),
                  _stream(dev, stream))
    return out


def selection_coefficient(obs, exp, alpha=None, theta=None, pi=None, device="cuda:0", stream=None):
    dev = torch.device(device)
    o, e = _dev(obs, torch.float64, dev).contiguous(), _dev(exp, torch.float64, dev).contiguous()
    want_p = alpha is not None
    a, t, p = ((_dev(x, torch.float64, dev).contiguous() for x in (alpha, theta, pi)) if want_p else (None, None, None))
    sel = torch.empty_like(o)
    pval = torch.empty_like(o) if want_p else None
    with torch.cuda.device(dev):
        _lib.call("dig_selection_coefficient", o.data_ptr(), e.data_ptr(), _ptr(a), _ptr(t), _ptr(p), o.numel(),
                  sel.data_ptr(), _ptr(pval), _stream(dev, stream))
    return sel, pval


def site_test(site_chrom, site_start, site_sub, site_k, window, win_map_off, win_map, win_counts, y_pred, std, d_pr,
              cj=1.0, site_strand=None, device="cuda:0", want=("P", "EXP"), stream=None, status_sink=None):
    dev = torch.device(device)
    sc, ss = _dev(site_chrom, torch.int32, dev), _dev(site_start, torch.int64, dev)
    sb, sk = _dev(site_sub, torch.uint8, dev), _dev(site_k, torch.float64, dev)
    st = _dev(site_strand, torch.int8, dev) if site_strand is not None else None
    wmo, wm = _dev(win_map_off, torch.int64, dev), _dev(win_map, torch.int32, dev)
    wc = _dev(win_counts, torch.int32, dev).contiguous()
    yp, sd = _dev(y_pred, torch.float64, dev).contiguous(), _dev(std, torch.float64, dev).contiguous()
    dp = _dev(d_pr, torch.float64, dev).contiguous()
    n_win, n = wc.shape[0], sc.numel()
    den_p = torch.empty(n_win, dtype=torch.float64, device=dev)
    den_m = torch.empty(n_win, dtype=torch.float64, device=dev)
    out = {"PVAL": torch.empty(n, dtype=torch.float64, device=dev)}
    for k in ("P", "EXP"):
        out[k] = torch.empty(n, dtype=torch.float64, device=dev) if k in want else None
    status = torch.zeros(1, dtype=torch.int32, device=dev)
    sptr = _stream(dev, stream)
    with torch.cuda.device(dev):
        _lib.call("dig_window_denominators", wc.data_ptr(), dp.data_ptr(), n_win, den_p.data_ptr(), den_m.data_ptr(), sptr)
        _lib.call("dig_site_test", sc.data_ptr(), ss.data_ptr(), sb.data_ptr(), _ptr(st), sk.data_ptr(), n, int(window),
                  int(wmo.numel()) - 1, wmo.data_ptr(), wm.data_ptr(), yp.data_ptr(), sd.data_ptr(), den_p.data_ptr(), den_m.data_ptr(),
                  dp.data_ptr(), float(cj), _ptr(out["P"]), _ptr(out["EXP"]), out["PVAL"].data_ptr(),
                  status.data_ptr(), sptr)
        _check_status(status, "dig_site_test", status_sink)
    out["DENOM_PLUS"], out["DENOM_MINUS"] = den_p, den_m
    return {k: v for k, v in out.items() if v is not None}


NB_MODES = {"greater": 0, "greater_midp": 1, "less": 2, "less_midp": 3, "exact": 4, "midp": 5}


def nb_pvalue_variant(mode, k, alpha, p, mu=None, device="cuda:0", stream=None):
    dev = torch.device(device)
    kk, aa, pp = (_dev(x, torch.float64, dev).contiguous() for x in (k, alpha, p))
    mm = _dev(mu, torch.float64, dev).contiguous() if mu is not None else None
    out = torch.empty_like(kk)
    with torch.cuda.device(dev):
        _lib.call("dig_nb_pvalue_variant", NB_MODES[mode], kk.data_ptr(), aa.data_ptr(), pp.data_ptr(), _ptr(mm),
                  kk.numel(), out.data_ptr(), _stream(dev, stream))
    return out


LL_KINDS = {"nb": 0, "pois": 1, "gamma": 2}


def loglik(kind, x, a, b=None, device="cuda:0", stream=None):
    dev = torch.device(device)
    xx, aa = _dev(x, torch.float64, dev).contiguous(), _dev(a, torch.float64, dev).contiguous()
    bb = _dev(b, torch.float64, dev).contiguous() if b is not None else None
    out = torch.empty_like(xx)
    with torch.cuda.device(dev):
        _lib.call("dig_loglik", LL_KINDS[kind], xx.data_ptr(), aa.data_ptr(), _ptr(bb), xx.numel(), out.data_ptr(),
                  _stream(dev, stream))
    return out


def gene_llr_test(model, alpha, theta, pi3, obs3, mrfold, t_syn=None, device="cuda:0", stream=None):
    dev = torch.device(device)
    a, t, m = (_dev(x, torch.float64, dev).contiguous() for x in (alpha, theta, mrfold))
    p3, o3 = _dev(pi3, torch.float64, dev).contiguous(), _dev(obs3, torch.float64, dev).contiguous()
    ts = _dev(t_syn, torch.float64, dev).contiguous() if t_syn is not None else None
    n = a.numel()
    assert p3.shape == (n, 3) and o3.shape == (n, 3)
    out = torch.empty((4, n), dtype=torch.float64, device=dev)
    with torch.cuda.device(dev):
        _lib.call("dig_gene_llr_test", {"nb": 0, "gamma_poisson": 1}[model], a.data_ptr(), t.data_ptr(), p3.data_ptr(),
                  o3.data_ptr(), m.data_ptr(), _ptr(ts), n, out.data_ptr(), _stream(dev, stream))
    return out


def overlap_pairs(blk_kstart, blk_kend, mut_kstart, mut_kend, device="cuda:0", stream=None):
    dev = torch.device(device)
    bks = np.asarray(blk_kstart, dtype=np.int64)
    order = np.argsort(bks, kind="stable")
    bks = bks[order]
    bke = np.asarray(blk_kend, dtype=np.int64)[order]
    pmax = np.maximum.accumulate(bke) if len(bke) else bke
    b0, b1, b2 = (_dev(x, torch.int64, dev) for x in (bks, bke, pmax))
    m0, m1 = _dev(mut_kstart, torch.int64, dev), _dev(mut_kend, torch.int64, dev)
    n_blk, n_mut = len(bks), m0.numel()
    sptr = _stream(dev, stream)
    off = torch.zeros(n_mut + 1, dtype=torch.int64, device=dev)
    with torch.cuda.device(dev):
        cnt = torch.zeros(max(n_mut, 1), dtype=torch.int64, device=dev)
        _lib.call("dig_overlap_count", _ptr(b0), _ptr(b1), _ptr(b2), n_blk, m0.data_ptr(), m1.data_ptr(), n_mut,
                  cnt.data_ptr(), sptr)
        off[1:] = torch.cumsum(cnt[:n_mut], 0)
        total = int(off[-1].item()) if n_mut else 0
        pm = torch.empty(max(total, 1), dtype=torch.int64, device=dev)
        pb = torch.empty(max(total, 1), dtype=torch.int64, device=dev)
        if total:
            _lib.call("dig_overlap_fill", b0.data_ptr(), b1.data_ptr(), b2.data_ptr(), n_blk, m0.data_ptr(),
                      m1.data_ptr(), n_mut, off.data_ptr(), pm.data_ptr(), pb.data_ptr(), sptr)
    return pm[:total].cpu().numpy(), order[pb[:total].cpu().numpy()]


def overlap_counts(blk_kstart, blk_kend, mut_kstart, mut_kend, device="cuda:0", stream=None):
    dev = torch.device(device)
    bks = np.asarray(blk_kstart, dtype=np.int64)
    order = np.argsort(bks, kind="stable")
    bks = bks[order]
    bke = np.asarray(blk_kend, dtype=np.int64)[order]
    pmax = np.maximum.accumulate(bke) if len(bke) else bke
    b0, b1, b2 = (_dev(x, torch.int64, dev) for x in (bks, bke, pmax))
    m0, m1 = _dev(mut_kstart, torch.int64, dev), _dev(mut_kend, torch.int64, dev)
    n_mut = m0.numel()
    cnt = torch.zeros(max(n_mut, 1), dtype=torch.int64, device=dev)
    with torch.cuda.device(dev):
        _lib.call("dig_overlap_count", _ptr(b0), _ptr(b1), _ptr(b2), len(bks), m0.data_ptr(), m1.data_ptr(), n_mut,
                  cnt.data_ptr(), _stream(dev, stream))
    return cnt[:n_mut].cpu().numpy()


def element_region_counts(elt_chrom, elt_strand, blk_ptr, blk_start, blk_end, window, win_map_off, win_map, win_counts,
                          device="cuda:0", stream=None, status_sink=None):
    dev = torch.device(device)
    ec, es = _dev(elt_chrom, torch.int32, dev), _dev(elt_strand, torch.int8, dev)
    bp, bs, be = (_dev(x, torch.int64, dev) for x in (blk_ptr, blk_start, blk_end))
    wmo, wm = _dev(win_map_off, torch.int64, dev), _dev(win_map, torch.int32, dev)
    wc = _dev(win_counts, torch.int32, dev).contiguous()
    n_elt = ec.numel()
    rc = torch.empty((max(n_elt, 1), 64), dtype=torch.int64, device=dev)
    nw = torch.empty(max(n_elt, 1), dtype=torch.int32, device=dev)
    status = torch.zeros(1, dtype=torch.int32, device=dev)
    with torch.cuda.device(dev):
        _lib.call("dig_element_region_counts", ec.data_ptr(), es.data_ptr(), bp.data_ptr(), bs.data_ptr(), be.data_ptr(),
                  n_elt, int(window), int(wmo.numel()) - 1, wmo.data_ptr(), wm.data_ptr(), wc.data_ptr(), wc.shape[0],
                  element_max_span(bp, bs, be, window), rc.data_ptr(), nw.data_ptr(), status.data_ptr(),
                  _stream(dev, stream))
        _check_status(status, "dig_element_region_counts", status_sink)
    return rc[:n_elt], nw[:n_elt]


def element_psum(L, region_counts, d_pr, device="cuda:0", stream=None, want_denom=False):
    dev = torch.device(device)
    Ld = _dev(L, torch.float64, dev).contiguous().reshape(-1, 192)
    Rd = _dev(region_counts, torch.int64, dev).contiguous().reshape(-1, 192)
    dp = _dev(d_pr, torch.float64, dev).contiguous()
    n = Ld.shape[0]
    assert Rd.shape[0] == n and dp.numel() == 192
    p = torch.empty(max(n, 1), dtype=torch.float64, device=dev)
    den = torch.empty(max(n, 1), dtype=torch.float64, device=dev) if want_denom else None
    with torch.cuda.device(dev):
        _lib.call("dig_element_psum", Ld.data_ptr(), Rd.data_ptr(), dp.data_ptr(), n, p.data_ptr(), _ptr(den),
                  _stream(dev, stream))
    return (p[:n], den[:n]) if want_denom else p[:n]



CDS_CLASS_NAMES = {0: "Synonymous", 1: "Missense", 2: "Nonsense", 3: "Essential_Splice", 5: "Stop_loss"}
CDS_NO_HIT = 255


def _splice_offsets(donor, acceptor):
    import ctypes
    d, a = [int(x) for x in donor], [int(x) for x in acceptor]
    return (ctypes.c_int32 * max(len(d), 1))(*d), len(d), (ctypes.c_int32 * max(len(a), 1))(*a), len(a)


def _check_cds_status(status, what):
    code = int(status.item())
    if code:
        why = [m for bit, m in ((1, "a gene has more than 2048 CDS blocks"),
                                (2, "a gene's chromosome or block lies outside the genome"),
                                (4, "a gene's blocks are not strictly ascending")) if code & bit]
        raise _lib.DigError("%s: %s" % (what, "; ".join(why)))


def cds_substitution_table(genome, gene_chrom, gene_strand, blk_ptr, blk_start, blk_end, donor=(1, 2, 5),
                           acceptor=(1, 2), stream=None):
    dev = genome.device
    gc, gs = _dev(gene_chrom, torch.int32, dev), _dev(gene_strand, torch.int8, dev)
    bp, bs, be = (_dev(x, torch.int64, dev) for x in (blk_ptr, blk_start, blk_end))
    E = gc.numel()
    L = torch.empty((max(E, 1), 192, 4), dtype=torch.float64, device=dev)
    flags = torch.empty(max(E, 1), dtype=torch.int32, device=dev)
    status = torch.zeros(1, dtype=torch.int32, device=dev)
    d, nd, a, na = _splice_offsets(donor, acceptor)
    with torch.cuda.device(dev):
        _lib.call("dig_cds_substitution_table", genome.packed2.data_ptr(), genome.nmask.data_ptr(), genome.n_bases,
                  genome.chrom_off_d.data_ptr(), genome.chrom_len_d.data_ptr(), len(genome.chrom_len), gc.data_ptr(),
                  gs.data_ptr(), bp.data_ptr(), bs.data_ptr(), be.data_ptr(), E, d, nd, a, na, L.data_ptr(),
                  flags.data_ptr(), status.data_ptr(), _stream(dev, stream))
        _check_cds_status(status, "dig_cds_substitution_table")
    return L[:E], flags[:E]


def annotate_snvs(genome, gene_chrom, gene_strand, blk_ptr, blk_start, blk_end, mut_chrom, mut_pos, mut_alt,
                  donor=(1, 2, 5), acceptor=(1, 2), stream=None):
    dev = genome.device
    gc, gs = _dev(gene_chrom, torch.int32, dev), _dev(gene_strand, torch.int8, dev)
    bp, bs, be = (_dev(x, torch.int64, dev) for x in (blk_ptr, blk_start, blk_end))
    mc, mp, ma = _dev(mut_chrom, torch.int64, dev), _dev(mut_pos, torch.int64, dev), _dev(mut_alt, torch.uint8, dev)
    E, n_mut = gc.numel(), mp.numel()
    pad = max([int(x) for x in donor] + [int(x) for x in acceptor] + [0])
    owner = torch.repeat_interleave(torch.arange(E, dtype=torch.int64, device=dev), bp[1:] - bp[:-1])
    kc = gc.to(torch.int64)[owner] << 32
    ks, order = torch.sort(kc | torch.clamp(bs - pad, min=0), stable=True)
    ke = (kc | (be + 1 + pad))[order]
    pmax = torch.cummax(ke, 0).values if ke.numel() else ke
    owner = owner[order]
    mks = (mc << 32) | mp
    mke = mks + 1
    sptr = _stream(dev, stream)
    empty = (torch.zeros(0, dtype=torch.int64, device=dev), torch.zeros(0, dtype=torch.int32, device=dev),
             torch.zeros(0, dtype=torch.uint8, device=dev))
    if n_mut == 0 or ks.numel() == 0:
        return empty
    with torch.cuda.device(dev):
        cnt = torch.empty(n_mut, dtype=torch.int64, device=dev)
        _lib.call("dig_overlap_count", ks.data_ptr(), ke.data_ptr(), pmax.data_ptr(), ks.numel(), mks.data_ptr(),
                  mke.data_ptr(), n_mut, cnt.data_ptr(), sptr)
        off = torch.zeros(n_mut + 1, dtype=torch.int64, device=dev)
        off[1:] = torch.cumsum(cnt, 0)
        total = int(off[-1].item())
        if total == 0:
            return empty
        pm = torch.empty(total, dtype=torch.int64, device=dev)
        pb = torch.empty(total, dtype=torch.int64, device=dev)
        _lib.call("dig_overlap_fill", ks.data_ptr(), ke.data_ptr(), pmax.data_ptr(), ks.numel(), mks.data_ptr(),
                  mke.data_ptr(), n_mut, off.data_ptr(), pm.data_ptr(), pb.data_ptr(), sptr)
        key = torch.unique(pm * E + owner[pb])
        pair_mut = torch.div(key, E, rounding_mode="floor")
        pair_gene = (key - pair_mut * E).to(torch.int32)
        cls = torch.empty(key.numel(), dtype=torch.uint8, device=dev)
        status = torch.zeros(1, dtype=torch.int32, device=dev)
        d, nd, a, na = _splice_offsets(donor, acceptor)
        _lib.call("dig_annotate_snvs", genome.packed2.data_ptr(), genome.nmask.data_ptr(), genome.n_bases,
                  genome.chrom_off_d.data_ptr(), genome.chrom_len_d.data_ptr(), len(genome.chrom_len), gc.data_ptr(),
                  gs.data_ptr(), bp.data_ptr(), bs.data_ptr(), be.data_ptr(), E, d, nd, a, na, mp.data_ptr(),
                  ma.data_ptr(), pair_mut.data_ptr(), pair_gene.data_ptr(), key.numel(), cls.data_ptr(),
                  status.data_ptr(), sptr)
        _check_cds_status(status, "dig_annotate_snvs")
    return pair_mut, pair_gene, cls
```

digdriver_b200/pipeline.py:

```python
from dataclasses import dataclass, field

import numpy as np
import torch

from . import kernels

GENE_CLASSES = ("SYN", "MIS", "NONS", "SPL", "TRUNC", "NONSYN")
ANNOT_CLASS = {"Synonymous": 0, "Missense": 1, "Nonsense": 2, "Essential_Splice": 3, "INDEL": 4}


def scan_windows(genome, win_chrom_idx, win_start, win_end, n_up, n_down, out=None, totals=None, stream=None):
    if totals is not None:
        totals.zero_()
    return kernels.count_contexts(genome, win_chrom_idx, win_start, win_end, n_up, n_down, want_totals=True,
                                  out=out, totals=totals, stream=stream)


def sequence_model(genome, mut_chrom_idx, mut_start, mut_ref, mut_alt, genome_totals64, n_up=1, n_down=1):
    ctx = kernels.mutation_contexts(genome, mut_chrom_idx, mut_start, mut_ref, n_up, n_down)
    counts = kernels.substitution_counts(ctx, mut_alt, n_up, n_down)
    denom = genome_totals64.to(torch.float64).repeat_interleave(3)
    return counts.to(torch.float64) / denom, counts, ctx


@dataclass
class GeneTable:
    chrom_idx: np.ndarray
    strand: np.ndarray
    blk_ptr: np.ndarray
    blk_start: np.ndarray
    blk_end: np.ndarray
    L: np.ndarray
    names: list = field(default_factory=list)
    tp53: int = -1
    cgc_mask: np.ndarray = None


def gene_pretrain(genes, window, win_map_off, win_map, win_counts64, y_pred, std, y_true, flag, d_pr,
                  device="cuda:0", cache=None):
    out = kernels.element_transfer(genes.chrom_idx, genes.strand, genes.blk_ptr, genes.blk_start, genes.blk_end,
                                   window, win_map_off, win_map, win_counts64, y_pred, std, y_true, flag, d_pr,
                                   L_elt=genes.L if cache is None else cache, device=device)
    return out


_CONST = {}


def _const_f64(value, device):
    key = (float(value), str(device))
    t = _CONST.get(key)
    if t is None:
        t = _CONST[key] = torch.full((1,), float(value), dtype=torch.float64, device=device)
    return t


def gene_burden_test(pre, obs, nsamp, n_syn_non_tp53, tp53=-1, cgc_mask=None, scale_factor=None, cohort=0,
                     collectives=None):
    mu, sigma = pre["MU"][cohort].contiguous(), pre["SIGMA"][cohort].contiguous()
    P = pre["P"][cohort].contiguous()
    pi_indel = kernels.size_ratio(pre["ELT_SIZE"], pre["R_SIZE"])
    sums = kernels.gene_scale_sums(mu, sigma, P, pi_indel, obs, cgc_mask, tp53)
    n_syn = float(n_syn_non_tp53)
    if collectives is not None and collectives.world > 1:
        sums = torch.cat([sums, _const_f64(n_syn, sums.device)])
        collectives.all_reduce_sum(sums)
        n_syn = None
    out = kernels.gene_burden_test(mu, sigma, P, pi_indel, obs, nsamp, sums, n_syn, scale_factor)
    res = {name: out[i] for i, name in enumerate(kernels.GENE_OUT_ROWS)}
    o = obs.to(torch.float64)
    res.update({"MU": mu, "SIGMA": sigma, "Pi_SYN": P[:, 0], "Pi_MIS": P[:, 1], "Pi_NONS": P[:, 2], "Pi_SPL": P[:, 3],
                "OBS_SYN": o[:, 0], "OBS_MIS": o[:, 1], "OBS_NONS": o[:, 2], "OBS_SPL": o[:, 3], "OBS_INDEL": o[:, 4],
                "SUMS": sums})
    return res


def element_burden_test(pre, obs, cj, cj_indel, cohort=0, skip_pvals=False):
    dev = obs.device
    E = obs.shape[0]
    mu, sigma = pre["MU"][cohort], pre["SIGMA"][cohort]
    pi_sum = pre["P"][cohort][:, 0]
    pi_indel = pre["ELT_SIZE"].to(torch.float64) / pre["R_SIZE"].to(torch.float64)
    alpha = mu ** 2 / sigma ** 2
    theta0 = sigma ** 2 / mu
    theta = theta0 * cj
    theta_indel = theta0 * cj_indel
    o = obs.to(torch.float64)
    res = {"ELT_SIZE": pre["ELT_SIZE"], "FLAG": pre["FLAG"][cohort], "R_SIZE": pre["R_SIZE"],
           "R_OBS": pre["R_OBS"][cohort], "R_INDEL": pre["R_OBS"][cohort], "MU": mu, "SIGMA": sigma,
           "ALPHA": alpha, "THETA": theta, "MU_INDEL": mu, "SIGMA_INDEL": sigma, "ALPHA_INDEL": alpha,
           "THETA_INDEL": theta_indel, "Pi_SUM": pi_sum, "Pi_INDEL": pi_indel,
           "OBS_SAMPLES": o[:, 0], "OBS_SNV": o[:, 1], "OBS_INDEL": o[:, 2]}
    if skip_pvals:
        res["EXP_SNV"] = alpha * theta * pi_sum
        return res
    kk = torch.stack([o[:, 1], o[:, 0], o[:, 2]])
    pp = torch.stack([pi_sum, pi_sum, pi_indel])
    tt = torch.stack([theta, theta, theta_indel])
    exp, pval = kernels.nb_burden_test(kk.reshape(-1), alpha.expand(3, E).reshape(-1), tt.reshape(-1),
                                       pp.reshape(-1), dev)
    exp, pval = exp.reshape(3, E), pval.reshape(3, E)
    res["EXP_SNV"] = exp[0]
    res["PVAL_SNV_BURDEN"] = pval[0]
    res["PVAL_SAMPLE_BURDEN"] = pval[1]
    if float(o[:, 2].sum()) != 0:
        res["EXP_INDEL"] = exp[2]
        res["PVAL_INDEL_BURDEN"] = pval[2]
        res["PVAL_MUT_BURDEN"] = kernels.fisher_combine2(pval[0], pval[2], dev)
    return res



def synth_region_params(n_win, seed):
    rng = np.random.default_rng(seed)
    y_pred = rng.gamma(2.0, 10.0, n_win)
    std = y_pred * rng.uniform(0.05, 0.5, n_win)
    y_true = rng.poisson(y_pred).astype(np.float64)
    flag = rng.random(n_win) < 0.1
    return y_pred, std, y_true, flag


def synth_genes(n_genes, chrom_lengths, window, seed):
    rng = np.random.default_rng(seed)
    chrom_lengths = np.asarray(chrom_lengths, dtype=np.int64)
    usable = np.maximum((chrom_lengths - 1) // window * window - 1, 0)
    p = usable / usable.sum()
    chrom = np.sort(rng.choice(len(chrom_lengths), size=n_genes, p=p)).astype(np.int32)
    nblk = np.minimum(1 + rng.geometric(1 / 8.7, n_genes), 300)
    ptr = np.zeros(n_genes + 1, dtype=np.int64)
    ptr[1:] = np.cumsum(nblk)
    tot = int(ptr[-1])
    exon = np.maximum(rng.lognormal(np.log(130.0), 0.7, tot).astype(np.int64), 3)
    intron = rng.lognormal(np.log(1500.0), 1.2, tot).astype(np.int64) + 20
    step = exon + intron
    owner = np.repeat(np.arange(n_genes), nblk)
    first = ptr[:-1][owner]
    cs = np.cumsum(step) - step
    rel = cs - cs[first]
    span = np.zeros(n_genes, dtype=np.int64)
    np.maximum.at(span, owner, rel + exon)
    g0 = (rng.random(n_genes) * np.maximum(usable[chrom] - span - 10, 1)).astype(np.int64) + 5
    start = g0[owner] + rel
    end = start + exon - 1
    lim = usable[chrom][owner] - 1
    start = np.minimum(start, lim - 1)
    end = np.minimum(np.maximum(end, start), lim)
    strand = np.where(rng.random(n_genes) < 0.5, -1, 1).astype(np.int8)
    return chrom, strand, ptr, start.astype(np.int64), end.astype(np.int64)


def synth_gene_L(blk_counts64, blk_ptr, seed):
    rng = np.random.default_rng(seed)
    E = len(blk_ptr) - 1
    owner = np.repeat(np.arange(E), np.diff(blk_ptr))
    L64 = np.zeros((E, 64), dtype=np.int64)
    np.add.at(L64, owner, np.asarray(blk_counts64, dtype=np.int64))
    L192 = np.repeat(L64, 3, axis=1).astype(np.float64)
    frac = rng.dirichlet([2.3, 6.8, 0.4, 0.5], size=192)
    L = np.floor(L192[:, :, None] * frac[None, :, :])
    return L
```

include/dig_b200.h:

```cpp
#ifndef DIG_B200_H
#define DIG_B200_H

#include <stdint.h>

#ifdef __cplusplus
extern "C" {
#endif

#define DIG_OK 0
#define DIG_ERR_ARG (-1)
#define DIG_ERR_CUDA (-2)
#define DIG_ERR_RANGE (-3)
#define DIG_ERR_UNSUPPORTED (-4)

int dig_version(void);
const char *dig_last_error(void);
int dig_device_sm_count(void);

int64_t dig_packed_words(int64_t n_bases);
int64_t dig_nmask_words(int64_t n_bases);
int dig_pack_genome(const uint8_t *ascii_d, int64_t n_bases, uint32_t *packed2_d, uint32_t *nmask_d,
                    unsigned long long *n_other_d, void *stream);

#define DIG_SCAN_AUTO 0
#define DIG_SCAN_PER_BASE 1
#define DIG_SCAN_HEX_PLAIN 2
#define DIG_SCAN_HEX 3
typedef struct dig_scan_opts {
    void *workspace_d;
    int64_t workspace_bytes;
    int32_t variant;
    uint32_t totals_limit_kb;
    int64_t tile_window;
    int32_t n_peer_counts3;
    int32_t nsum_offset_words;
    void *peer_counts3_d[8];
    void *mc_counts3_d;
} dig_scan_opts;
int64_t dig_scan_workspace_bytes(int64_t n_reg);

int dig_count_contexts(const uint32_t *packed2_d, const uint32_t *nmask_d, int64_t n_bases,
                       const int64_t *chrom_off_d, const int64_t *chrom_len_d,
                       const int32_t *reg_chrom_d, const int64_t *reg_start_d, const int64_t *reg_end_d,
                       const int8_t *reg_strand_d, int64_t n_reg, int n_up, int n_down,
                       int32_t *counts_d, unsigned long long *totals_d, const dig_scan_opts *opts, void *stream);

int dig_count_contexts_fused53(const uint32_t *packed2_d, const uint32_t *nmask_d, int64_t n_bases,
                               const int64_t *chrom_off_d, const int64_t *chrom_len_d,
                               const int32_t *reg_chrom_d, const int64_t *reg_start_d, const int64_t *reg_end_d,
                               int64_t n_reg, int32_t *counts5_d, int32_t *counts3_d,
                               unsigned long long *totals5_d, unsigned long long *totals3_d,
                               const dig_scan_opts *opts, void *stream);

int dig_narrow_counts_u16(const int32_t *counts_d, int64_t n_values, uint16_t *out_d, int32_t *status_d, void *stream);

int dig_nmask_fill_runs(const int64_t *runs_d, int64_t n_runs, uint32_t *nmask_d, int64_t word0, int64_t n_words, void *stream);

int dig_nmask_summary(const uint32_t *nmask_d, int64_t word0, int64_t n_words, uint32_t *nsum_d, void *stream);

int dig_peer_broadcast(const void *src_d, int64_t nbytes, void *const *dst_d, int n_dst, void *stream);

int dig_mutation_contexts(const uint32_t *packed2_d, const uint32_t *nmask_d, int64_t n_bases,
                          const int64_t *chrom_off_d, const int64_t *chrom_len_d,
                          const int32_t *mut_chrom_d, const int64_t *mut_start_d, const uint8_t *mut_ref_d,
                          int64_t n_mut, int n_up, int n_down, int32_t *ctx_out_d, void *stream);

int dig_substitution_counts(const int32_t *ctx_d, const uint8_t *alt_d, int64_t n, int n_up, int n_down,
                            unsigned long long *counts_d, void *stream);

int64_t dig_tabulate_capacity(int64_t n_pairs);
int64_t dig_tabulate_elements_workspace_bytes(int64_t n_pairs);
int64_t dig_tabulate_genes_workspace_bytes(int64_t n_mut);
int dig_count_hits(const int64_t *blk_kstart_d, const int64_t *blk_kend_d, const int64_t *blk_pmax_d,
                   const int32_t *blk_elt_d, int64_t n_blk, const int64_t *mut_kstart_d,
                   const int64_t *mut_kend_d, int64_t n_mut, unsigned long long *n_hits_d, void *stream);
int dig_tabulate_elements(const int64_t *blk_kstart_d, const int64_t *blk_kend_d, const int64_t *blk_pmax_d,
                          const int32_t *blk_elt_d, int64_t n_blk, const int64_t *mut_kstart_d,
                          const int64_t *mut_kend_d, const int32_t *mut_sample_d, const uint8_t *mut_isindel_d,
                          int64_t n_mut, unsigned long long *tab_key_d, uint32_t *tab_snv_d,
                          uint32_t *tab_indel_d, int64_t capacity, int64_t n_sample,
                          unsigned long long *sample_tot_d, int64_t max_muts_per_sample,
                          int64_t max_per_elt_per_sample, int64_t n_elt, int64_t *obs_d, int32_t *status_d,
                          int sample_rows_mode, void *stream);

int dig_site_counts(const int32_t *site_elt_d, const int32_t *site_sub_d, int64_t n_site, int64_t n_elt, int n_sub,
                    unsigned long long *L_d, void *stream);

int dig_tabulate_genes(const int32_t *mut_gene_d, const int32_t *mut_sample_d, const uint8_t *mut_class_d,
                       int64_t n_mut, unsigned long long *tab_key_d, uint32_t *tab_cnt_d, int64_t capacity,
                       int64_t max_per_gene_per_sample, int64_t n_gene, int64_t *obs_d, int64_t *nsamp_d,
                       int32_t *status_d, void *stream);

int dig_element_transfer(const int32_t *elt_chrom_d, const int8_t *elt_strand_d, const int64_t *blk_ptr_d,
                         const int64_t *blk_start_d, const int64_t *blk_end_d, int64_t n_elt, int64_t window,
                         int n_chrom, const int64_t *win_map_off_d, const int32_t *win_map_d,
                         const int32_t *win_counts_d, const double *y_pred_d, const double *std_d, const double *y_true_d,
                         const uint8_t *flag_d, int64_t n_win, int n_cohort, const double *d_pr_d,
                         const int32_t *blk_counts_d, const double *L_elt_d, int n_col, int max_span_windows,
                         double *mu_d, double *sigma_d, double *r_obs_d, uint8_t *flag_out_d, int64_t *r_size_d,
                         int64_t *elt_size_d, double *p_out_d, int32_t *n_win_out_d, int32_t *status_d,
                         void *stream);

int dig_nb_pvalue_greater_midp(const double *k_d, const double *alpha_d, const double *p_d, int64_t n,
                               double *pval_out_d, void *stream);
int dig_nb_burden_test(const double *k_d, const double *alpha_d, const double *theta_d, const double *pi_d,
                       int64_t n, double *exp_out_d, double *pval_out_d, void *stream);
int dig_fisher_combine2(const double *p1_d, const double *p2_d, int64_t n, double *out_d, void *stream);

int dig_sequence_freq(const unsigned long long *subst_counts_d, const unsigned long long *ctx_totals_d, int n_ctx,
                      double *freq_d, void *stream);
int dig_size_ratio(const int64_t *num_d, const int64_t *den_d, int64_t n, double *out_d, void *stream);
int dig_gene_scale_sums(const double *mu_d, const double *sigma_d, const double *p_d, const double *pi_indel_d,
                        const int64_t *obs_d, const uint8_t *cgc_mask_d, int64_t tp53, int64_t n_gene,
                        double *sums_d, void *stream);
int dig_gene_burden_test(const double *mu_d, const double *sigma_d, const double *p_d, const double *pi_indel_d,
                         const int64_t *obs_d, const int64_t *nsamp_d, int64_t n_gene, const double *sums_d,
                         double n_syn, double scale_factor, double *out_d, void *stream);

int dig_gene_dnds_sel(const double *alpha_d, const double *theta_d, const double *pi6_d, const double *obs6_d,
                      int64_t n_gene, double *out_d, void *stream);
int dig_selection_coefficient(const double *obs_d, const double *exp_d, const double *alpha_d, const double *theta_d,
                              const double *pi_d, int64_t n, double *sel_d, double *pval_d, void *stream);

int dig_window_denominators(const int32_t *win_counts_d, const double *d_pr_d, int64_t n_win, double *denom_plus_d,
                            double *denom_minus_d, void *stream);
int dig_site_test(const int32_t *site_chrom_d, const int64_t *site_start_d, const uint8_t *site_sub_d,
                  const int8_t *site_strand_d, const double *site_k_d, int64_t n_site, int64_t window, int n_chrom,
                  const int64_t *win_map_off_d, const int32_t *win_map_d, const double *y_pred_d, const double *std_d,
                  const double *denom_plus_d, const double *denom_minus_d, const double *d_pr_d, double cj,
                  double *p_out_d, double *exp_out_d, double *pval_out_d, int32_t *status_d, void *stream);

int dig_region_prob_norm(const int32_t *counts_d, const double *s_prob_d, int64_t n_reg, int n_ctx, double *norm_d,
                         void *stream);
int dig_position_obs(const int64_t *mut_key_d, int64_t n_mut, const int64_t *chrom_off_d, const int64_t *chrom_len_d,
                     const int32_t *reg_chrom_d, const int64_t *reg_start_d, const int64_t *reg_end_d, int64_t n_reg,
                     int n_up, int n_down, int binsize, const int64_t *bin_ptr_d, int64_t n_bin, int32_t *obs_d,
                     void *stream);
int dig_position_test(const uint32_t *packed2_d, const uint32_t *nmask_d, int64_t n_bases, const int64_t *chrom_off_d,
                      const int64_t *chrom_len_d, const int32_t *reg_chrom_d, const int64_t *reg_start_d,
                      const int64_t *reg_end_d, int64_t n_reg, int n_up, int n_down, const double *s_prob_d,
                      const double *norm_d, const double *mu_d, const double *sigma_d, int binsize,
                      const int64_t *bin_ptr_d, const int32_t *obs_d, double *pval_d, double *pt_d, double *exp_d,
                      double *pos_d, void *stream);
int dig_nb_pvalue_exact(const double *k_d, const double *alpha_d, const double *p_d, int64_t n, double *pval_out_d,
                        void *stream);

#define DIG_NB_GREATER 0
#define DIG_NB_GREATER_MIDP 1
#define DIG_NB_LESS 2
#define DIG_NB_LESS_MIDP 3
#define DIG_NB_EXACT 4
#define DIG_NB_MIDP 5
int dig_nb_pvalue_variant(int mode, const double *k_d, const double *alpha_d, const double *p_d, const double *mu_d,
                          int64_t n, double *pval_out_d, void *stream);

#define DIG_LL_NB 0
#define DIG_LL_POIS 1
#define DIG_LL_GAMMA 2
int dig_loglik(int kind, const double *x_d, const double *a_d, const double *b_d, int64_t n, double *out_d, void *stream);

#define DIG_LLR_NB 0
#define DIG_LLR_GAMMA_POISSON 1
int dig_gene_llr_test(int model, const double *alpha_d, const double *theta_d, const double *pi3_d, const double *obs3_d,
                      const double *mrfold_d, const double *t_syn_d, int64_t n, double *out_d, void *stream);

int dig_overlap_count(const int64_t *blk_kstart_d, const int64_t *blk_kend_d, const int64_t *blk_pmax_d, int64_t n_blk,
                      const int64_t *mut_kstart_d, const int64_t *mut_kend_d, int64_t n_mut, int64_t *n_pairs_d,
                      void *stream);
int dig_overlap_fill(const int64_t *blk_kstart_d, const int64_t *blk_kend_d, const int64_t *blk_pmax_d, int64_t n_blk,
                     const int64_t *mut_kstart_d, const int64_t *mut_kend_d, int64_t n_mut, const int64_t *pair_off_d,
                     int64_t *pair_mut_d, int64_t *pair_blk_d, void *stream);

int dig_element_region_counts(const int32_t *elt_chrom_d, const int8_t *elt_strand_d, const int64_t *blk_ptr_d,
                              const int64_t *blk_start_d, const int64_t *blk_end_d, int64_t n_elt, int64_t window,
                              int n_chrom, const int64_t *win_map_off_d, const int32_t *win_map_d,
                              const int32_t *win_counts_d, int64_t n_win, int max_span_windows, int64_t *region_counts_d, int32_t *n_win_out_d,
                              int32_t *status_d, void *stream);

int dig_element_psum(const double *L_d, const int64_t *region_counts_d, const double *d_pr_d, int64_t n_elt,
                     double *p_out_d, double *denom_out_d, void *stream);

#define DIG_CDS_SYNONYMOUS 0
#define DIG_CDS_MISSENSE 1
#define DIG_CDS_NONSENSE 2
#define DIG_CDS_ESSENTIAL_SPLICE 3
#define DIG_CDS_STOP_LOSS 5
#define DIG_CDS_NO_HIT 255
#define DIG_CDS_FLAG_LENGTH 1
#define DIG_CDS_FLAG_N 2
#define DIG_CDS_FLAG_STOP 4
#define DIG_CDS_ERR_BLOCKS 1
#define DIG_CDS_ERR_RANGE 2
#define DIG_CDS_ERR_ORDER 4
#define DIG_CDS_MAX_BLOCKS 2048
#define DIG_CDS_MAX_SPLICE_OFFSETS 8
int dig_cds_substitution_table(const uint32_t *packed2_d, const uint32_t *nmask_d, int64_t n_bases,
                               const int64_t *chrom_off_d, const int64_t *chrom_len_d, int n_chrom,
                               const int32_t *gene_chrom_d, const int8_t *gene_strand_d, const int64_t *blk_ptr_d,
                               const int64_t *blk_start_d, const int64_t *blk_end_d, int64_t n_gene,
                               const int32_t *donor, int n_donor, const int32_t *acceptor, int n_acceptor,
                               double *L_d, int32_t *flags_d, int32_t *status_d, void *stream);
int dig_annotate_snvs(const uint32_t *packed2_d, const uint32_t *nmask_d, int64_t n_bases,
                      const int64_t *chrom_off_d, const int64_t *chrom_len_d, int n_chrom,
                      const int32_t *gene_chrom_d, const int8_t *gene_strand_d, const int64_t *blk_ptr_d,
                      const int64_t *blk_start_d, const int64_t *blk_end_d, int64_t n_gene,
                      const int32_t *donor, int n_donor, const int32_t *acceptor, int n_acceptor,
                      const int64_t *mut_pos_d, const uint8_t *mut_alt_d, const int64_t *pair_mut_d,
                      const int32_t *pair_gene_d, int64_t n_pair, uint8_t *class_out_d, int32_t *status_d,
                      void *stream);

int dig_synth_genome(uint8_t *ascii_d, int64_t g0, int64_t n, uint64_t seed, int n_frac16, void *stream);

#ifdef __cplusplus
}
#endif
#endif
```

Measured before the change: 2822 billion.

## Add programmatic dependent launch and fold small follow-up kernels into producers

Kernels are now launched with CUDA programmatic stream serialization (griddepcontrol wait/trigger), so each launch can overlap the tail of the one before it. Several launches and memsets go away: the gene Fisher combine is done by the last arriving thread through an atomic counter, the substitution histogram uses a self-resetting scratch buffer instead of a memset, pi_indel is computed inside element transfer, and the OBS rows are written by the gene test kernel. Status words and hash tables are reused as pre-zeroed buffers. This cuts launch and host overhead but adds atomics, fences and persistent scratch state that must stay zeroed between calls.

```diff
diff --git a/digdriver_b200/_lib.py b/digdriver_b200/_lib.py
--- a/digdriver_b200/_lib.py
+++ b/digdriver_b200/_lib.py
@@ -15,6 +15,7 @@
     "dig_version": (_I, []),
     "dig_last_error": (_c.c_char_p, []),
     "dig_device_sm_count": (_I, []),
+    "dig_set_pdl": (_I, [_I]),
     "dig_packed_words": (_I64, [_I64]),
     "dig_nmask_words": (_I64, [_I64]),
     "dig_pack_genome": (_I, [_P, _I64, _P, _P, _P, _P]),
@@ -30,21 +31,21 @@
     "dig_tabulate_genes_workspace_bytes": (_I64, [_I64]),
     "dig_synth_genome": (_I, [_P, _I64, _I64, _U64, _I, _P]),
     "dig_mutation_contexts": (_I, [_P, _P, _I64, _P, _P, _P, _P, _P, _I64, _I, _I, _P, _P]),
-    "dig_substitution_counts": (_I, [_P, _P, _I64, _I, _I, _P, _P]),
+    "dig_substitution_counts": (_I, [_P, _P, _I64, _I, _I, _P, _P, _P]),
     "dig_count_hits": (_I, [_P, _P, _P, _P, _I64, _P, _P, _I64, _P, _P]),
     "dig_tabulate_elements": (_I, [_P, _P, _P, _P, _I64, _P, _P, _P, _P, _I64, _P, _P, _P, _I64, _I64, _P,
                                    _I64, _I64, _I64, _P, _P, _I, _P]),
     "dig_site_counts": (_I, [_P, _P, _I64, _I64, _I, _P, _P]),
-    "dig_tabulate_genes": (_I, [_P, _P, _P, _I64, _P, _P, _I64, _I64, _I64, _P, _P, _P, _P]),
+    "dig_tabulate_genes": (_I, [_P, _P, _P, _I64, _P, _P, _I64, _I64, _I64, _P, _P, _P, _I, _P]),
     "dig_element_transfer": (_I, [_P, _P, _P, _P, _P, _I64, _I64, _I, _P, _P, _P, _P, _P, _P, _P, _I64, _I, _P,
-                                  _P, _P, _I, _I, _P, _P, _P, _P, _P, _P, _P, _P, _P, _P]),
+                                  _P, _P, _I, _I, _P, _P, _P, _P, _P, _P, _P, _P, _P, _P, _P]),
     "dig_nb_pvalue_greater_midp": (_I, [_P, _P, _P, _I64, _P, _P]),
     "dig_nb_burden_test": (_I, [_P, _P, _P, _P, _I64, _P, _P, _P]),
     "dig_fisher_combine2": (_I, [_P, _P, _I64, _P, _P]),
     "dig_sequence_freq": (_I, [_P, _P, _I, _P, _P]),
     "dig_size_ratio": (_I, [_P, _P, _I64, _P, _P]),
     "dig_gene_scale_sums": (_I, [_P, _P, _P, _P, _P, _P, _I64, _I64, _P, _P]),
-    "dig_gene_burden_test": (_I, [_P, _P, _P, _P, _P, _P, _I64, _P, _D, _D, _P, _P]),
+    "dig_gene_burden_test": (_I, [_P, _P, _P, _P, _P, _P, _I64, _P, _D, _D, _P, _P, _P]),
     "dig_gene_dnds_sel": (_I, [_P, _P, _P, _P, _I64, _P, _P]),
     "dig_selection_coefficient": (_I, [_P, _P, _P, _P, _P, _I64, _P, _P, _P]),
     "dig_window_denominators": (_I, [_P, _P, _I64, _P, _P, _P]),
@@ -83,7 +84,7 @@
     "dig_pack_genome": 1, "dig_count_contexts": 1, "dig_count_contexts_fused53": 1, "dig_synth_genome": 1, "dig_mutation_contexts": 1,
     "dig_substitution_counts": 1, "dig_count_hits": 1, "dig_tabulate_elements": 3, "dig_tabulate_genes": 2, "dig_site_counts": 1,
     "dig_element_transfer": 1, "dig_nb_pvalue_greater_midp": 1, "dig_nb_burden_test": 1, "dig_fisher_combine2": 1,
-    "dig_sequence_freq": 1, "dig_size_ratio": 1, "dig_gene_scale_sums": 1, "dig_gene_burden_test": 2,
+    "dig_sequence_freq": 1, "dig_size_ratio": 1, "dig_gene_scale_sums": 1, "dig_gene_burden_test": 1,
     "dig_window_denominators": 1, "dig_site_test": 1, "dig_gene_dnds_sel": 1, "dig_selection_coefficient": 1, "dig_region_prob_norm": 1, "dig_position_obs": 1, "dig_position_test": 1, "dig_nb_pvalue_exact": 1,
     "dig_nb_pvalue_variant": 1, "dig_loglik": 1, "dig_gene_llr_test": 1, "dig_overlap_count": 1, "dig_overlap_fill": 1,
     "dig_element_region_counts": 1, "dig_element_psum": 1, "dig_narrow_counts_u16": 1, "dig_peer_broadcast": 1, "dig_nmask_fill_runs": 1,
diff --git a/digdriver_b200/csrc/api.cu b/digdriver_b200/csrc/api.cu
--- a/digdriver_b200/csrc/api.cu
+++ b/digdriver_b200/csrc/api.cu
@@ -1,4 +1,5 @@
 #include <stdarg.h>
+#include <stdlib.h>
 #include <string.h>
 
 #include "dig_common.cuh"
@@ -30,9 +31,27 @@
     return cached;
 }
 
+static int g_pdl = -1;
+
+bool pdl_enabled()
+{
+    if (g_pdl < 0) {
+        const char *v = getenv("DIG_NO_PDL");
+        g_pdl = (v != nullptr && v[0] != '\0' && strcmp(v, "0") != 0) ? 0 : 1;
+    }
+    return g_pdl != 0;
+}
+
 }
 
 extern "C" {
+
+int dig_set_pdl(int enabled)
+{
+    const int prev = dig::pdl_enabled() ? 1 : 0;
+    dig::g_pdl = enabled ? 1 : 0;
+    return prev;
+}
 
 int dig_version(void) { return 100; }
 
diff --git a/digdriver_b200/csrc/dig_common.cuh b/digdriver_b200/csrc/dig_common.cuh
--- a/digdriver_b200/csrc/dig_common.cuh
+++ b/digdriver_b200/csrc/dig_common.cuh
@@ -10,7 +10,28 @@
 void set_error(const char *fmt, ...);
 int sm_count();
 
-#define DIG_CHECK_ARG(cond, msg)                           \
+bool pdl_enabled();
+
+__device__ __forceinline__ void pdl_wait() { asm volatile("griddepcontrol.wait;" ::: "memory"); }
+__device__ __forceinline__ void pdl_trigger() { asm volatile("griddepcontrol.launch_dependents;" ::: "memory"); }
+
+template <typename... KArgs, typename... Args>
+cudaError_t launch_pdl(void (*kernel)(KArgs...), dim3 grid, dim3 block, size_t smem, cudaStream_t st, Args &&...args)
+{
+    cudaLaunchAttribute attr[1];
+    attr[0].id = cudaLaunchAttributeProgrammaticStreamSerialization;
+    attr[0].val.programmaticStreamSerializationAllowed = 1;
+    cudaLaunchConfig_t cfg = {};
+    cfg.gridDim = grid;
+    cfg.blockDim = block;
+    cfg.dynamicSmemBytes = smem;
+    cfg.stream = st;
+    cfg.attrs = attr;
+    cfg.numAttrs = pdl_enabled() ? 1 : 0;
+    return cudaLaunchKernelEx(&cfg, kernel, static_cast<KArgs>(args)...);
+}
+
+#define DIG_CHECK_ARG(cond, msg)                         \
     do {                                                   \
         if (!(cond)) {                                     \
             dig::set_error("%s: %s", __func__, msg);       \
diff --git a/digdriver_b200/csrc/genetest.cu b/digdriver_b200/csrc/genetest.cu
--- a/digdriver_b200/csrc/genetest.cu
+++ b/digdriver_b200/csrc/genetest.cu
@@ -16,6 +16,7 @@
     cooperative_groups::cluster_group cluster = cooperative_groups::this_cluster();
     const unsigned int rank = cluster.block_rank();
     double a0 = 0.0, a1 = 0.0, a2 = 0.0;
+    dig::pdl_wait();
 #pragma unroll 4
     for (int64_t g = (int64_t)rank * 1024 + threadIdx.x; g < n; g += (int64_t)SUMS_CLUSTER * 1024) {
         const double m = mu[g], s = sigma[g];
@@ -29,6 +30,7 @@
             a2 += (double)obs[g * 5 + 4];
         }
     }
+    dig::pdl_trigger();
     sh[0][threadIdx.x] = a0;
     sh[1][threadIdx.x] = a1;
     sh[2][threadIdx.x] = a2;
@@ -54,9 +56,10 @@
     const double *__restrict__ mu, const double *__restrict__ sigma, const double *__restrict__ P,
     const double *__restrict__ pi_indel, const int64_t *__restrict__ obs, const int64_t *__restrict__ nsamp,
     int64_t n, const double *__restrict__ sums, double n_syn,
-    double scale_factor, double *__restrict__ out)
-{
-    const int64_t stride = (int64_t)gridDim.x * blockDim.x;
+    double scale_factor, double *__restrict__ out, unsigned int *__restrict__ arrive)
+{
+    const int64_t stride = (int64_t)gridDim.x * blockDim.x;
+    dig::pdl_wait();
     const double cj = isnan(scale_factor) ? (isnan(n_syn) ? sums[3] : n_syn) / sums[0] : scale_factor;
     const double t_indel = sums[2] / sums[1];
     for (int64_t i = (int64_t)blockIdx.x * blockDim.x + threadIdx.x; i < n * 13; i += stride) {
@@ -68,6 +71,7 @@
         const double p_syn = P[g * 4 + 0], p_mis = P[g * 4 + 1], p_nons = P[g * 4 + 2], p_spl = P[g * 4 + 3];
         const double p_trunc = p_nons + p_spl;
         const double p_nonsyn = p_mis + p_trunc;
+        dig::pdl_trigger();
         double pi, k, theta;
         if (t == 12) {
             pi = pi_indel[g];
@@ -104,6 +108,16 @@
             out[24 * n + g] = pi_indel[g];
             out[25 * n + g] = p_trunc;
             out[26 * n + g] = p_nonsyn;
+#pragma unroll
+            for (int j = 0; j < 5; ++j) out[(int64_t)(27 + j) * n + g] = (double)obs[g * 5 + j];
+        }
+        if (arrive != nullptr && (t == 4 || t == 12)) {
+            __threadfence();
+            if (atomicAdd(arrive + g, 1u) == 1u) {
+                __threadfence();
+                out[20 * n + g] = fisher2(__ldcg(out + (6 + 4) * n + g), __ldcg(out + 19 * n + g));
+                arrive[g] = 0u;
+            }
         }
     }
 }
@@ -111,6 +125,7 @@
 __global__ void __launch_bounds__(256) gene_fisher_kernel(int64_t n, double *__restrict__ out)
 {
     const int64_t stride = (int64_t)gridDim.x * blockDim.x;
+    dig::pdl_wait();
     for (int64_t g = (int64_t)blockIdx.x * blockDim.x + threadIdx.x; g < n; g += stride)
         out[20 * n + g] = fisher2(out[(6 + 4) * n + g], out[19 * n + g]);
 }
@@ -120,6 +135,7 @@
                                                        double *__restrict__ freq)
 {
     const int j = blockIdx.x * blockDim.x + threadIdx.x;
+    dig::pdl_wait();
     if (j < n_sub) freq[j] = (double)counts[j] / (double)totals[j / 3];
 }
 
@@ -149,8 +165,8 @@
 {
     DIG_CHECK_ARG(n_ctx > 0 && subst_counts_d && ctx_totals_d && freq_d, "bad arguments");
     const int n_sub = 3 * n_ctx;
-    seq_freq_kernel<<<(n_sub + 255) / 256, 256, 0, (cudaStream_t)stream>>>(subst_counts_d, ctx_totals_d, n_sub, freq_d);
-    DIG_CHECK_LAUNCH();
+    DIG_CUDA(dig::launch_pdl(seq_freq_kernel, dim3((n_sub + 255) / 256), dim3(256), 0, (cudaStream_t)stream, subst_counts_d,
+                             ctx_totals_d, n_sub, freq_d));
     return DIG_OK;
 }
 
@@ -160,15 +176,14 @@
 {
     DIG_CHECK_ARG(n_gene >= 0 && sums_d, "bad arguments");
     DIG_CHECK_ARG(n_gene == 0 || (mu_d && sigma_d && p_d && pi_indel_d && obs_d), "null pointer");
-    gene_scale_sums_kernel<<<SUMS_CLUSTER, 1024, 0, (cudaStream_t)stream>>>(mu_d, sigma_d, p_d, pi_indel_d, obs_d, cgc_mask_d,
-                                                                 tp53, n_gene, sums_d);
-    DIG_CHECK_LAUNCH();
+    DIG_CUDA(dig::launch_pdl(gene_scale_sums_kernel, dim3(SUMS_CLUSTER), dim3(1024), 0, (cudaStream_t)stream, mu_d, sigma_d,
+                             p_d, pi_indel_d, obs_d, cgc_mask_d, tp53, n_gene, sums_d));
     return DIG_OK;
 }
 
 int dig_gene_burden_test(const double *mu_d, const double *sigma_d, const double *p_d, const double *pi_indel_d,
                          const int64_t *obs_d, const int64_t *nsamp_d, int64_t n_gene, const double *sums_d,
-                         double n_syn, double scale_factor, double *out_d, void *stream)
+                         double n_syn, double scale_factor, double *out_d, unsigned int *arrive_d, void *stream)
 {
     DIG_CHECK_ARG(n_gene >= 0, "negative size");
     if (n_gene == 0) return DIG_OK;
@@ -177,11 +192,10 @@
     int64_t blocks = (n_gene * 13 + 127) / 128;
     const int64_t cap = (int64_t)dig::sm_count() * 32;
     if (blocks > cap) blocks = cap;
-    gene_test_kernel<<<(unsigned)blocks, 128, 0, st>>>(mu_d, sigma_d, p_d, pi_indel_d, obs_d, nsamp_d, n_gene, sums_d,
-                                                       n_syn, scale_factor, out_d);
-    DIG_CHECK_LAUNCH();
-    gene_fisher_kernel<<<(unsigned)((n_gene + 255) / 256), 256, 0, st>>>(n_gene, out_d);
-    DIG_CHECK_LAUNCH();
+    DIG_CUDA(dig::launch_pdl(gene_test_kernel, dim3((unsigned)blocks), dim3(128), 0, st, mu_d, sigma_d, p_d, pi_indel_d, obs_d,
+                             nsamp_d, n_gene, sums_d, n_syn, scale_factor, out_d, arrive_d));
+    if (arrive_d == nullptr)
+        DIG_CUDA(dig::launch_pdl(gene_fisher_kernel, dim3((unsigned)((n_gene + 255) / 256)), dim3(256), 0, st, n_gene, out_d));
     return DIG_OK;
 }
 
diff --git a/digdriver_b200/csrc/mutctx.cu b/digdriver_b200/csrc/mutctx.cu
--- a/digdriver_b200/csrc/mutctx.cu
+++ b/digdriver_b200/csrc/mutctx.cu
@@ -10,11 +10,13 @@
 {
     const int klen = n_up + n_down + 1;
     const int64_t stride = (int64_t)gridDim.x * blockDim.x;
+    dig::pdl_wait();
     for (int64_t i = (int64_t)blockIdx.x * blockDim.x + threadIdx.x; i < n_mut; i += stride) {
         const int32_t c = mut_chrom[i];
         const int64_t p = mut_start[i];
         const int64_t L = __ldg(chrom_len + c);
         const int64_t off = __ldg(chrom_off + c);
+        dig::pdl_trigger();
         int32_t ctx = -1;
         if (p - n_up >= 0 && p + n_down < L) {
             const int64_t f = off + p - n_up;
@@ -40,11 +42,14 @@
 
 __global__ void __launch_bounds__(256) subst_hist_kernel(const int32_t *__restrict__ ctx,
                                                          const uint8_t *__restrict__ alt, int64_t n, int n_down,
-                                                         int n_bins, unsigned long long *__restrict__ counts)
+                                                         int n_bins, unsigned long long *__restrict__ counts,
+                                                         unsigned long long *__restrict__ scratch)
 {
     extern __shared__ unsigned int sh[];
+    __shared__ bool last;
     for (int k = threadIdx.x; k < n_bins; k += blockDim.x) sh[k] = 0u;
     __syncthreads();
+    dig::pdl_wait();
     const int64_t stride = (int64_t)gridDim.x * blockDim.x;
     for (int64_t i = (int64_t)blockIdx.x * blockDim.x + threadIdx.x; i < n; i += stride) {
         const int32_t c = ctx[i];
@@ -54,30 +59,43 @@
         if (a == ref) continue;
         atomicAdd(sh + 3 * c + (int)(a > ref ? a - 1u : a), 1u);
     }
+    dig::pdl_trigger();
     __syncthreads();
+    unsigned long long *dst = scratch != nullptr ? scratch : counts;
     for (int k = threadIdx.x; k < n_bins; k += blockDim.x)
-        if (sh[k]) atomicAdd(counts + k, (unsigned long long)sh[k]);
+        if (sh[k]) atomicAdd(dst + k, (unsigned long long)sh[k]);
+    if (scratch == nullptr) return;
+    __threadfence();
+    __syncthreads();
+    if (threadIdx.x == 0) last = atomicAdd(scratch + n_bins, 1ull) == (unsigned long long)gridDim.x - 1ull;
+    __syncthreads();
+    if (!last) return;
+    __threadfence();
+    for (int k = threadIdx.x; k < n_bins; k += blockDim.x) {
+        counts[k] = __ldcg(scratch + k);
+        scratch[k] = 0ull;
+    }
+    if (threadIdx.x == 0) scratch[n_bins] = 0ull;
 }
 
 }
 
 extern "C" int dig_substitution_counts(const int32_t *ctx_d, const uint8_t *alt_d, int64_t n, int n_up, int n_down,
-                                       unsigned long long *counts_d, void *stream)
+                                       unsigned long long *counts_d, unsigned long long *scratch_d, void *stream)
 {
     DIG_CHECK_ARG(n >= 0, "negative size");
     DIG_CHECK_ARG(n_up >= 0 && n_down >= 0 && n_up + n_down <= 5, "unsupported context size");
     DIG_CHECK_ARG(counts_d != nullptr, "null pointer");
     const int n_bins = 3 << (2 * (n_up + n_down + 1));
     cudaStream_t st = (cudaStream_t)stream;
-    DIG_CUDA(cudaMemsetAsync(counts_d, 0, (size_t)n_bins * sizeof(unsigned long long), st));
+    if (n == 0 || scratch_d == nullptr) DIG_CUDA(cudaMemsetAsync(counts_d, 0, (size_t)n_bins * sizeof(unsigned long long), st));
     if (n == 0) return DIG_OK;
     DIG_CHECK_ARG(ctx_d && alt_d, "null pointer");
     int64_t blocks = (n + 255) / 256;
     const int64_t cap = (int64_t)dig::sm_count() * 4;
     if (blocks > cap) blocks = cap;
-    subst_hist_kernel<<<(unsigned)blocks, 256, (size_t)n_bins * sizeof(unsigned int), st>>>(ctx_d, alt_d, n, n_down,
-                                                                                          n_bins, counts_d);
-    DIG_CHECK_LAUNCH();
+    DIG_CUDA(dig::launch_pdl(subst_hist_kernel, dim3((unsigned)blocks), dim3(256), (size_t)n_bins * sizeof(unsigned int), st,
+                             ctx_d, alt_d, n, n_down, n_bins, counts_d, scratch_d));
     return DIG_OK;
 }
 
@@ -96,9 +114,8 @@
     int64_t blocks = (n_mut + 255) / 256;
     const int64_t cap = (int64_t)dig::sm_count() * 32;
     if (blocks > cap) blocks = cap;
-    mutctx_kernel<<<(unsigned)blocks, 256, 0, (cudaStream_t)stream>>>(
-        packed2_d, nmask_d, (((n_bases + 31) >> 5) << 1) - 1, ((n_bases + 31) >> 5) - 1, chrom_off_d, chrom_len_d,
-        mut_chrom_d, mut_start_d, mut_ref_d, n_mut, n_up, n_down, ctx_out_d);
-    DIG_CHECK_LAUNCH();
+    DIG_CUDA(dig::launch_pdl(mutctx_kernel, dim3((unsigned)blocks), dim3(256), 0, (cudaStream_t)stream, packed2_d, nmask_d,
+                             (((n_bases + 31) >> 5) << 1) - 1, ((n_bases + 31) >> 5) - 1, chrom_off_d, chrom_len_d,
+                             mut_chrom_d, mut_start_d, mut_ref_d, n_mut, n_up, n_down, ctx_out_d));
     return DIG_OK;
 }
diff --git a/digdriver_b200/csrc/obs.cu b/digdriver_b200/csrc/obs.cu
--- a/digdriver_b200/csrc/obs.cu
+++ b/digdriver_b200/csrc/obs.cu
@@ -123,6 +123,7 @@
                                                           int32_t *status)
 {
     const int64_t stride = (int64_t)gridDim.x * blockDim.x;
+    dig::pdl_wait();
     for (int64_t i = (int64_t)blockIdx.x * blockDim.x + threadIdx.x; i < n_mut; i += stride) {
         const uint32_t cls = mclass[i];
         const int32_t g = mgene[i];
@@ -138,20 +139,26 @@
     }
 }
 
-__global__ void __launch_bounds__(256) gene_finalize_kernel(const unsigned long long *__restrict__ keys,
-                                                            const uint32_t *__restrict__ cnt, int64_t capacity,
+__global__ void __launch_bounds__(256) gene_finalize_kernel(unsigned long long *__restrict__ keys,
+                                                            uint32_t *__restrict__ cnt, int64_t capacity,
                                                             int64_t cap_per, int64_t n_gene, int64_t *obs,
-                                                            int64_t *nsamp)
-{
-    const int64_t stride = (int64_t)gridDim.x * blockDim.x;
+                                                            int64_t *nsamp, int clear)
+{
+    const int64_t stride = (int64_t)gridDim.x * blockDim.x;
+    dig::pdl_wait();
     for (int64_t s = (int64_t)blockIdx.x * blockDim.x + threadIdx.x; s < capacity; s += stride) {
         const unsigned long long key = keys[s];
         if (key == 0ull) continue;
+        int64_t c[5];
+#pragma unroll
+        for (int j = 0; j < 5; ++j) c[j] = cnt[s * 5 + j];
+        if (clear) {
+            keys[s] = 0ull;
+#pragma unroll
+            for (int j = 0; j < 5; ++j) cnt[s * 5 + j] = 0u;
+        }
         const int64_t g = (int64_t)((key - 1ull) >> 32);
         if (g >= n_gene) continue;
-        int64_t c[5];
-#pragma unroll
-        for (int j = 0; j < 5; ++j) c[j] = cnt[s * 5 + j];
 #pragma unroll
         for (int j = 0; j < 5; ++j) {
             const int64_t v = c[j] > cap_per ? cap_per : c[j];
@@ -294,14 +301,16 @@
 int dig_tabulate_genes(const int32_t *mut_gene_d, const int32_t *mut_sample_d, const uint8_t *mut_class_d,
                        int64_t n_mut, unsigned long long *tab_key_d, uint32_t *tab_cnt_d, int64_t capacity,
                        int64_t max_per_gene_per_sample, int64_t n_gene, int64_t *obs_d, int64_t *nsamp_d,
-                       int32_t *status_d, void *stream)
+                       int32_t *status_d, int table_zeroed, void *stream)
 {
     DIG_CHECK_ARG(n_mut >= 0 && n_gene >= 0, "negative size");
     DIG_CHECK_ARG(is_pow2(capacity), "capacity must be a power of two");
     DIG_CHECK_ARG(tab_key_d && tab_cnt_d && status_d && (n_gene == 0 || (obs_d && nsamp_d)), "null pointer");
     cudaStream_t st = (cudaStream_t)stream;
-    DIG_CUDA(cudaMemsetAsync(tab_key_d, 0, (size_t)capacity * sizeof(unsigned long long), st));
-    DIG_CUDA(cudaMemsetAsync(tab_cnt_d, 0, (size_t)capacity * 5 * sizeof(uint32_t), st));
+    if (!table_zeroed) {
+        DIG_CUDA(cudaMemsetAsync(tab_key_d, 0, (size_t)capacity * sizeof(unsigned long long), st));
+        DIG_CUDA(cudaMemsetAsync(tab_cnt_d, 0, (size_t)capacity * 5 * sizeof(uint32_t), st));
+    }
     DIG_CUDA(cudaMemsetAsync(status_d, 0, sizeof(int32_t), st));
     if (n_gene) {
         DIG_CUDA(cudaMemsetAsync(obs_d, 0, (size_t)n_gene * 5 * sizeof(int64_t), st));
@@ -309,12 +318,10 @@
     }
     if (n_mut == 0) return DIG_OK;
     DIG_CHECK_ARG(mut_gene_d && mut_sample_d && mut_class_d, "null pointer");
-    gene_insert_kernel<<<grid_for(n_mut), 256, 0, st>>>(mut_gene_d, mut_sample_d, mut_class_d, n_mut, tab_key_d,
-                                                        tab_cnt_d, capacity, status_d);
-    DIG_CHECK_LAUNCH();
-    gene_finalize_kernel<<<grid_for(capacity), 256, 0, st>>>(tab_key_d, tab_cnt_d, capacity,
-                                                             max_per_gene_per_sample, n_gene, obs_d, nsamp_d);
-    DIG_CHECK_LAUNCH();
+    DIG_CUDA(dig::launch_pdl(gene_insert_kernel, dim3(grid_for(n_mut)), dim3(256), 0, st, mut_gene_d, mut_sample_d,
+                             mut_class_d, n_mut, tab_key_d, tab_cnt_d, capacity, status_d));
+    DIG_CUDA(dig::launch_pdl(gene_finalize_kernel, dim3(grid_for(capacity)), dim3(256), 0, st, tab_key_d, tab_cnt_d,
+                             capacity, max_per_gene_per_sample, n_gene, obs_d, nsamp_d, table_zeroed));
     return DIG_OK;
 }
 
diff --git a/digdriver_b200/csrc/transfer.cu b/digdriver_b200/csrc/transfer.cu
--- a/digdriver_b200/csrc/transfer.cu
+++ b/digdriver_b200/csrc/transfer.cu
@@ -32,8 +32,8 @@
     const int32_t *__restrict__ blk_counts, const double *__restrict__ L_elt, int n_col, int span_words,
     double *__restrict__ mu_out, double *__restrict__ sigma_out, double *__restrict__ robs_out,
     uint8_t *__restrict__ flag_out, int64_t *__restrict__ r_size, int64_t *__restrict__ elt_size,
-    double *__restrict__ p_out, int32_t *__restrict__ n_win_out, int32_t *__restrict__ status,
-    int64_t *__restrict__ region_counts_out)
+    double *__restrict__ p_out, int32_t *__restrict__ n_win_out, double *__restrict__ pi_indel_out,
+    int32_t *__restrict__ status, int64_t *__restrict__ region_counts_out)
 {
     extern __shared__ __align__(16) unsigned char smem_raw[];
     const int lane = threadIdx.x & 31;
@@ -46,6 +46,7 @@
     const bool l4_aligned = (reinterpret_cast<uintptr_t>(L_elt) & 15u) == 0;
     const int64_t gwarp = (int64_t)blockIdx.x * TW + warp;
     const int64_t nwarps = (int64_t)gridDim.x * TW;
+    dig::pdl_wait();
 
     for (int64_t e = gwarp; e < n_elt; e += nwarps) {
         const int64_t b0 = blk_ptr[e], b1 = blk_ptr[e + 1];
@@ -169,6 +170,7 @@
                 }
             }
         }
+        dig::pdl_trigger();
         __syncwarp();
         if (!minus) {
             r64[lane] = r_lo;
@@ -265,8 +267,11 @@
             }
         }
         if (lane == 0) {
-            if (!RC || r_size) r_size[e] = (int64_t)rsum;
-            if (!RC || elt_size) elt_size[e] = blk_counts != nullptr ? (int64_t)lsum : gene_len;
+            const int64_t rs = (int64_t)rsum;
+            const int64_t es = blk_counts != nullptr ? (int64_t)lsum : gene_len;
+            if (!RC || r_size) r_size[e] = rs;
+            if (!RC || elt_size) elt_size[e] = es;
+            if (pi_indel_out != nullptr) pi_indel_out[e] = __ddiv_rn((double)es, (double)rs);
             n_win_out[e] = nw;
         }
         __syncwarp();
@@ -283,7 +288,7 @@
                                     const double *d_pr_d, const int32_t *blk_counts_d, const double *L_elt_d,
                                     int n_col, int max_span_windows, double *mu_d, double *sigma_d, double *r_obs_d,
                                     uint8_t *flag_out_d, int64_t *r_size_d, int64_t *elt_size_d, double *p_out_d,
-                                    int32_t *n_win_out_d, int32_t *status_d, void *stream)
+                                    int32_t *n_win_out_d, double *pi_indel_d, int32_t *status_d, void *stream)
 {
     DIG_CHECK_ARG(n_elt >= 0 && n_win >= 0 && window > 0 && n_chrom >= 0, "bad sizes");
     DIG_CHECK_ARG(n_cohort >= 1 && n_cohort <= 32 * MAX_COHORT_PER_LANE, "n_cohort must be in [1, 64] per call");
@@ -292,7 +297,6 @@
     DIG_CHECK_ARG(n_col >= 1 && max_span_windows >= 1, "bad n_col / max_span_windows");
     DIG_CHECK_ARG(status_d != nullptr, "null pointer");
     cudaStream_t st = (cudaStream_t)stream;
-    DIG_CUDA(cudaMemsetAsync(status_d, 0, sizeof(int32_t), st));
     if (n_elt == 0) return DIG_OK;
     DIG_CHECK_ARG(elt_chrom_d && elt_strand_d && blk_ptr_d && blk_start_d && blk_end_d && win_map_off_d &&
                       win_map_d && win_counts_d && y_pred_d && std_d && y_true_d && flag_d && d_pr_d && mu_d &&
@@ -309,11 +313,11 @@
     int64_t blocks = (n_elt + TW - 1) / TW;
     const int64_t cap = (int64_t)dig::sm_count() * 64;
     if (blocks > cap) blocks = cap;
-    transfer_kernel<false><<<(unsigned)blocks, TW * 32, smem, st>>>(
-        elt_chrom_d, elt_strand_d, blk_ptr_d, blk_start_d, blk_end_d, n_elt, window, n_chrom, win_map_off_d, win_map_d,
-        win_counts_d, y_pred_d, std_d, y_true_d, flag_d, n_win, n_cohort, d_pr_d, blk_counts_d, L_elt_d, n_col,
-        span_words, mu_d, sigma_d, r_obs_d, flag_out_d, r_size_d, elt_size_d, p_out_d, n_win_out_d, status_d, nullptr);
-    DIG_CHECK_LAUNCH();
+    DIG_CUDA(dig::launch_pdl(transfer_kernel<false>, dim3((unsigned)blocks), dim3(TW * 32), smem, st, elt_chrom_d,
+                             elt_strand_d, blk_ptr_d, blk_start_d, blk_end_d, n_elt, window, n_chrom, win_map_off_d,
+                             win_map_d, win_counts_d, y_pred_d, std_d, y_true_d, flag_d, n_win, n_cohort, d_pr_d,
+                             blk_counts_d, L_elt_d, n_col, span_words, mu_d, sigma_d, r_obs_d, flag_out_d, r_size_d,
+                             elt_size_d, p_out_d, n_win_out_d, pi_indel_d, status_d, nullptr));
     return DIG_OK;
 }
 
@@ -342,11 +346,11 @@
     int64_t blocks = (n_elt + TW - 1) / TW;
     const int64_t cap = (int64_t)dig::sm_count() * 64;
     if (blocks > cap) blocks = cap;
-    transfer_kernel<true><<<(unsigned)blocks, TW * 32, smem, st>>>(
-        elt_chrom_d, elt_strand_d, blk_ptr_d, blk_start_d, blk_end_d, n_elt, window, n_chrom, win_map_off_d, win_map_d,
-        win_counts_d, nullptr, nullptr, nullptr, nullptr, n_win, 0, nullptr, nullptr, nullptr, 0, span_words, nullptr,
-        nullptr, nullptr, nullptr, nullptr, nullptr, nullptr, n_win_out_d, status_d, region_counts_d);
-    DIG_CHECK_LAUNCH();
+    DIG_CUDA(dig::launch_pdl(transfer_kernel<true>, dim3((unsigned)blocks), dim3(TW * 32), smem, st, elt_chrom_d,
+                             elt_strand_d, blk_ptr_d, blk_start_d, blk_end_d, n_elt, window, n_chrom, win_map_off_d,
+                             win_map_d, win_counts_d, nullptr, nullptr, nullptr, nullptr, n_win, 0, nullptr, nullptr,
+                             nullptr, 0, span_words, nullptr, nullptr, nullptr, nullptr, nullptr, nullptr, nullptr,
+                             n_win_out_d, nullptr, status_d, region_counts_d));
     return DIG_OK;
 }
 
diff --git a/digdriver_b200/kernels.py b/digdriver_b200/kernels.py
--- a/digdriver_b200/kernels.py
+++ b/digdriver_b200/kernels.py
@@ -166,6 +166,34 @@
     return out
 
 
+_ZEROED = {}
+_ZEROED_RETIRED = []
+
+
+def _zeroed(name, n, dtype, device):
+    dev = torch.device(device)
+    if dev.index is None:
+        dev = torch.device("cuda", torch.cuda.current_device())
+    key = (name, dev.index)
+    t = _ZEROED.get(key)
+    if t is None or t.numel() < n:
+        if torch.cuda.is_current_stream_capturing():
+            return None
+        if t is not None:
+            _ZEROED_RETIRED.append(t)
+        t = _ZEROED[key] = torch.zeros(max(n, 1), dtype=dtype, device=dev)
+    return t[:n]
+
+
+def _status_word(what, device):
+    st = _zeroed("status:" + what, 1, torch.int32, device)
+    return st if st is not None else torch.zeros(1, dtype=torch.int32, device=device)
+
+
+def set_pdl(enabled):
+    return bool(_lib.load().dig_set_pdl(int(bool(enabled))))
+
+
 def _table_capacity(n_pairs):
     return int(_lib.load().dig_tabulate_capacity(int(n_pairs)))
 
@@ -175,6 +203,8 @@
         sink.append((status, what))
         return
     code = int(status.item())
+    if code != 0:
+        status.zero_()
     if code == 1:
         raise _lib.DigError("%s: hash table overflow" % what)
     if code == 2:
@@ -241,14 +271,18 @@
     n_mut = mg.numel()
     cap = _table_capacity(n_mut)
     with torch.cuda.device(dev):
-        keys = torch.empty(cap, dtype=torch.int64, device=dev)
-        cnt = torch.empty((cap, 5), dtype=torch.int32, device=dev)
+        table = _zeroed("tabulate_genes:%d" % cap, cap * 7, torch.int32, dev)
+        if table is not None:
+            keys, cnt = table[: 2 * cap].view(torch.int64), table[2 * cap:].view(cap, 5)
+        else:
+            keys = torch.empty(cap, dtype=torch.int64, device=dev)
+            cnt = torch.empty((cap, 5), dtype=torch.int32, device=dev)
         obs = torch.empty((max(n_gene, 1), 5), dtype=torch.int64, device=dev)
         nsamp = torch.empty((max(n_gene, 1), 7), dtype=torch.int64, device=dev)
-        status = torch.zeros(1, dtype=torch.int32, device=dev)
+        status = _status_word("dig_tabulate_genes", dev)
         _lib.call("dig_tabulate_genes", mg.data_ptr(), ms.data_ptr(), mc.data_ptr(), n_mut, keys.data_ptr(),
                   cnt.data_ptr(), cap, int(min(max_per_gene_per_sample, 2 ** 62)), n_gene, obs.data_ptr(),
-                  nsamp.data_ptr(), status.data_ptr(), _stream(dev, stream))
+                  nsamp.data_ptr(), status.data_ptr(), int(table is not None), _stream(dev, stream))
         _check_status(status, "dig_tabulate_genes", status_sink)
     return obs[:n_gene], nsamp[:n_gene]
 
@@ -287,14 +321,16 @@
         "P": torch.empty((n_cohort, n_elt, n_col), dtype=torch.float64, device=dev),
         "N_WIN": torch.empty(n_elt, dtype=torch.int32, device=dev),
     }
-    status = torch.zeros(1, dtype=torch.int32, device=dev)
+    if bc is None:
+        out["PI_INDEL"] = torch.empty(n_elt, dtype=torch.float64, device=dev)
+    status = _status_word("dig_element_transfer", dev)
     with torch.cuda.device(dev):
         _lib.call("dig_element_transfer", ec.data_ptr(), es.data_ptr(), bp.data_ptr(), bs.data_ptr(), be.data_ptr(),
                   n_elt, int(window), int(wmo.numel()) - 1, wmo.data_ptr(), wm.data_ptr(), wc.data_ptr(), yp.data_ptr(),
                   sd.data_ptr(), yt.data_ptr(), fl.data_ptr(), n_win, n_cohort, dp.data_ptr(), _ptr(bc), _ptr(Le), n_col, max_span,
                   out["MU"].data_ptr(), out["SIGMA"].data_ptr(), out["R_OBS"].data_ptr(), out["FLAG"].data_ptr(),
                   out["R_SIZE"].data_ptr(), out["ELT_SIZE"].data_ptr(), out["P"].data_ptr(),
-                  out["N_WIN"].data_ptr(), status.data_ptr(), _stream(dev, stream))
+                  out["N_WIN"].data_ptr(), _ptr(out.get("PI_INDEL")), status.data_ptr(), _stream(dev, stream))
         _check_status(status, "dig_element_transfer", status_sink)
     return out
 
@@ -337,10 +373,12 @@
     al = _dev(alt, torch.uint8, dev)
     if out is None:
         out = torch.empty(3 * 4 ** (n_up + n_down + 1), dtype=torch.int64, device=dev)
-    assert out.dtype == torch.int64 and out.is_contiguous() and out.numel() == 3 * 4 ** (n_up + n_down + 1)
+    n_bins = 3 * 4 ** (n_up + n_down + 1)
+    assert out.dtype == torch.int64 and out.is_contiguous() and out.numel() == n_bins
+    scratch = _zeroed("subst_counts:%d" % n_bins, n_bins + 1, torch.int64, dev)
     with torch.cuda.device(dev):
         _lib.call("dig_substitution_counts", ctx.data_ptr(), al.data_ptr(), ctx.numel(), int(n_up), int(n_down),
-                  out.data_ptr(), _stream(dev, stream))
+                  out.data_ptr(), _ptr(scratch), _stream(dev, stream))
     return out
 
 
@@ -358,7 +396,8 @@
                  ["PVAL_%s_BURDEN" % c for c in ("SYN", "MIS", "NONS", "SPL", "TRUNC", "NONSYN")] +
                  ["PVAL_%s_BURDEN_SAMPLE" % c for c in ("SYN", "MIS", "NONS", "SPL", "TRUNC", "NONSYN")] +
                  ["EXP_INDEL", "PVAL_INDEL_BURDEN", "PVAL_MUT_BURDEN", "ALPHA", "THETA", "THETA_INDEL", "Pi_INDEL",
-                  "Pi_TRUNC", "Pi_NONSYN"])
+                  "Pi_TRUNC", "Pi_NONSYN"] +
+                 ["OBS_" + c for c in ("SYN", "MIS", "NONS", "SPL", "INDEL")])
 
 
 def size_ratio(num, den, stream=None):
@@ -385,10 +424,12 @@
     dev = mu.device
     E = mu.numel()
     out = torch.empty((len(GENE_OUT_ROWS), E), dtype=torch.float64, device=dev)
+    arrive = _zeroed("fisher_arrive", E, torch.int32, dev)
     with torch.cuda.device(dev):
         _lib.call("dig_gene_burden_test", mu.data_ptr(), sigma.data_ptr(), P.data_ptr(), pi_indel.data_ptr(),
                   obs.data_ptr(), nsamp.data_ptr(), E, sums.data_ptr(), float("nan") if n_syn is None else float(n_syn),
-                  float("nan") if scale_factor is None else float(scale_factor), out.data_ptr(), _stream(dev, stream))
+                  float("nan") if scale_factor is None else float(scale_factor), out.data_ptr(), _ptr(arrive),
+                  _stream(dev, stream))
     return out
 
 
diff --git a/digdriver_b200/pipeline.py b/digdriver_b200/pipeline.py
--- a/digdriver_b200/pipeline.py
+++ b/digdriver_b200/pipeline.py
@@ -59,7 +59,7 @@
                      collectives=None):
     mu, sigma = pre["MU"][cohort].contiguous(), pre["SIGMA"][cohort].contiguous()
     P = pre["P"][cohort].contiguous()
-    pi_indel = kernels.size_ratio(pre["ELT_SIZE"], pre["R_SIZE"])
+    pi_indel = pre["PI_INDEL"]
     sums = kernels.gene_scale_sums(mu, sigma, P, pi_indel, obs, cgc_mask, tp53)
     n_syn = float(n_syn_non_tp53)
     if collectives is not None and collectives.world > 1:
@@ -68,9 +68,7 @@
         n_syn = None
     out = kernels.gene_burden_test(mu, sigma, P, pi_indel, obs, nsamp, sums, n_syn, scale_factor)
     res = {name: out[i] for i, name in enumerate(kernels.GENE_OUT_ROWS)}
-    o = obs.to(torch.float64)
     res.update({"MU": mu, "SIGMA": sigma, "Pi_SYN": P[:, 0], "Pi_MIS": P[:, 1], "Pi_NONS": P[:, 2], "Pi_SPL": P[:, 3],
-                "OBS_SYN": o[:, 0], "OBS_MIS": o[:, 1], "OBS_NONS": o[:, 2], "OBS_SPL": o[:, 3], "OBS_INDEL": o[:, 4],
                 "SUMS": sums})
     return res
 
diff --git a/include/dig_b200.h b/include/dig_b200.h
--- a/include/dig_b200.h
+++ b/include/dig_b200.h
@@ -16,6 +16,7 @@
 int dig_version(void);
 const char *dig_last_error(void);
 int dig_device_sm_count(void);
+int dig_set_pdl(int enabled);
 
 int64_t dig_packed_words(int64_t n_bases);
 int64_t dig_nmask_words(int64_t n_bases);
@@ -66,7 +67,7 @@
                           int64_t n_mut, int n_up, int n_down, int32_t *ctx_out_d, void *stream);
 
 int dig_substitution_counts(const int32_t *ctx_d, const uint8_t *alt_d, int64_t n, int n_up, int n_down,
-                            unsigned long long *counts_d, void *stream);
+                            unsigned long long *counts_d, unsigned long long *scratch_d, void *stream);
 
 int64_t dig_tabulate_capacity(int64_t n_pairs);
 int64_t dig_tabulate_elements_workspace_bytes(int64_t n_pairs);
@@ -89,7 +90,7 @@
 int dig_tabulate_genes(const int32_t *mut_gene_d, const int32_t *mut_sample_d, const uint8_t *mut_class_d,
                        int64_t n_mut, unsigned long long *tab_key_d, uint32_t *tab_cnt_d, int64_t capacity,
                        int64_t max_per_gene_per_sample, int64_t n_gene, int64_t *obs_d, int64_t *nsamp_d,
-                       int32_t *status_d, void *stream);
+                       int32_t *status_d, int table_zeroed, void *stream);
 
 int dig_element_transfer(const int32_t *elt_chrom_d, const int8_t *elt_strand_d, const int64_t *blk_ptr_d,
                          const int64_t *blk_start_d, const int64_t *blk_end_d, int64_t n_elt, int64_t window,
@@ -98,8 +99,8 @@
                          const uint8_t *flag_d, int64_t n_win, int n_cohort, const double *d_pr_d,
                          const int32_t *blk_counts_d, const double *L_elt_d, int n_col, int max_span_windows,
                          double *mu_d, double *sigma_d, double *r_obs_d, uint8_t *flag_out_d, int64_t *r_size_d,
-                         int64_t *elt_size_d, double *p_out_d, int32_t *n_win_out_d, int32_t *status_d,
-                         void *stream);
+                         int64_t *elt_size_d, double *p_out_d, int32_t *n_win_out_d, double *pi_indel_d,
+                         int32_t *status_d, void *stream);
 
 int dig_nb_pvalue_greater_midp(const double *k_d, const double *alpha_d, const double *p_d, int64_t n,
                                double *pval_out_d, void *stream);
@@ -115,7 +116,7 @@
                         double *sums_d, void *stream);
 int dig_gene_burden_test(const double *mu_d, const double *sigma_d, const double *p_d, const double *pi_indel_d,
                          const int64_t *obs_d, const int64_t *nsamp_d, int64_t n_gene, const double *sums_d,
-                         double n_syn, double scale_factor, double *out_d, void *stream);
+                         double n_syn, double scale_factor, double *out_d, unsigned int *arrive_d, void *stream);
 
 int dig_gene_dnds_sel(const double *alpha_d, const double *theta_d, const double *pi6_d, const double *obs6_d,
                       int64_t n_gene, double *out_d, void *stream);
```

Measured after the change: 2607 billion (median of 6 runs). 7.6% lower.
